# YoungSeng/QPGesture

Measured on AMD Instinct MI355X. Metric: matched gesture frames/sec (GestureKNN), higher is better.
Workload: dtype split-f16 products / f64 block sums + f64 re-evaluation; 1 GPU; 1 x 24 s clip (M=6 windows, Q=48 steps, 1440 frames each) per job vs speaker-10-class DB N_db=2048 windows (53248 candidates), shipped mode wavlm_feat(f32-bounded/f64-exact)+text(f32)+phase; n_db=2048, windows_per_clip=6, clips=1, clips_per_gpu=1, feature_dtype=f32, audio_precision=mixed, encode_batch=0, clips_in_flight=1, parallelism=single GPU, unsharded DB

## Files before the change

include/qpg.h:

```cpp
#ifndef QPG_H
#define QPG_H

#include <stddef.h>
#include <stdint.h>

#ifdef __cplusplus
extern "C" {
#endif

#define QPG_OK 0
#define QPG_EINVAL (-1)
#define QPG_EHIP (-2)
#define QPG_EUNSUP (-3)

typedef struct qpg_ctx qpg_ctx;

int qpg_version(void);
const char* qpg_build_id(void);
int qpg_ctx_create(int device, qpg_ctx** out);
int qpg_dev_kernarg(void);
int qpg_ctx_destroy(qpg_ctx* ctx);
#define QPG_OPT_GATE_DEDUP_FROM_CHAINS 0
#define QPG_OPT_TAKES_STAGES 1
#define QPG_OPT_COUNT 4
int qpg_ctx_set_option(qpg_ctx* ctx, int option, int value);
int qpg_ctx_get_option(qpg_ctx* ctx, int option, int* value);
int qpg_last_error(char* buf, size_t n);
int qpg_signal_i32(qpg_ctx*, void* stream, int32_t* dst, int32_t value);
int qpg_doorbell_wait(qpg_ctx*, void* stream, int32_t* counter, const int32_t* go, int32_t timeout_ms);


int qpg_wavlm_resample_f32(qpg_ctx*, void* stream, const float* x, int64_t N, int Tin, int F, int Tout, float* out);

int qpg_frame_norm2_f64(qpg_ctx*, void* stream, const float* x, int64_t rows, int F, double* out);

int qpg_audio_cand_norm2(qpg_ctx*, void* stream, const double* fn2, int N, int T, const int32_t* cand_t,
                         int G, int n_taps, int tap_stride, double* cn2);

int qpg_l2_normalize_rows_f32(qpg_ctx*, void* stream, const float* x, int64_t rows, int D, float* out);
int qpg_text_pack_queries_f32(qpg_ctx*, void* stream, const float* x, int M, int R, int D, const int32_t* q_win,
                              const int32_t* q_row, int Q, float* out);


int qpg_audio_pack_queries(qpg_ctx*, void* stream, const float* qbase, int M, int T, int F,
                           const int32_t* q_win, const int32_t* q_t, int Q, int n_taps, int tap_stride,
                           float* q32, double* qn2);

int qpg_audio_cosine_f64(qpg_ctx*, void* stream, const float* base, int N, int T, int F,
                         const int32_t* cand_t, int G, int n_taps, int tap_stride, const double* cn2,
                         const float* q32, const double* qn2, int Q, double* D, int64_t ldD);
int qpg_audio_cosine_f64_h(qpg_ctx*, void* stream, const void* base_f16, int N, int T, int F,
                           const int32_t* cand_t, int G, int n_taps, int tap_stride, const double* cn2,
                           const float* q32, const double* qn2, int Q, double* D, int64_t ldD);

#define QPG_AUDIO_MX_ERR 2.05e-6
int qpg_audio_cosine_mx(qpg_ctx*, void* stream, const float* base, int N, int T, int F, const int32_t* cand_t, int G,
                        int n_taps, int tap_stride, const double* cn2, const float* q32, const double* qn2, int Q,
                        void* D, int d_is_f32, int64_t ldD, int32_t* stats);

int qpg_audio_cosine_mx_h(qpg_ctx*, void* stream, const void* base_f16, int N, int T, int F, const int32_t* cand_t, int G,
                          int n_taps, int tap_stride, const double* cn2, const float* q32, const double* qn2, int Q,
                          void* D, int d_is_f32, int64_t ldD, int32_t* stats);

#define QPG_AUDIO_HL_ERR 1.3e-6
int qpg_audio_hl_supported(int T, int F, int G, int n_taps, int tap_stride, int cand_step);
int qpg_audio_pack_queries_hl(qpg_ctx*, void* stream, const float* qbase, int M, int T, int F, const int32_t* q_win,
                              const int32_t* q_t, int Q, int n_taps, int tap_stride, float* q32, double* qn2, void* image,
                              int64_t image_bytes);
int64_t qpg_audio_hl_db_bytes(int N, int F);
int64_t qpg_audio_hl_query_bytes(int Q, int F);
int qpg_audio_hl_pack_db(qpg_ctx*, void* stream, const float* base, int N, int T, int F, int G, int n_taps, int tap_stride,
                         int cand_step, void* image, int64_t image_bytes);
int qpg_audio_hl_pack_queries(qpg_ctx*, void* stream, const float* q32, int Q, int F, void* image, int64_t image_bytes);
int qpg_clip_pack_hl(qpg_ctx*, void* stream, const float* qbase, int M, int T, int F, const int32_t* q_win,
                     const int32_t* q_t, int Q, int n_taps, int tap_stride, float* q32, double* qn2, void* image,
                     int64_t image_bytes, const float* text_ctx, int Mt, int R, int Dt, const int32_t* tq_win,
                     const int32_t* tq_row, int Qt, float* qn_out, void* cols_image, int64_t cols_bytes);
int qpg_audio_cosine_hl(qpg_ctx*, void* stream, const void* db_image, int N, int F, int G, const double* cn2,
                        const void* q_image, const double* qn2, int Q, void* D, int d_is_f32, int64_t ldD, int32_t* stats);
int qpg_audio_hl1_supported(int T, int F, int G, int n_taps, int tap_stride, int cand_step);
int64_t qpg_audio_hl1_db_bytes(int N, int F);
int qpg_audio_hl1_pack_db(qpg_ctx*, void* stream, const void* base_f16, int N, int T, int F, int G, int n_taps,
                          int tap_stride, int cand_step, void* image, int64_t image_bytes);
int qpg_audio_cosine_hl1(qpg_ctx*, void* stream, const void* db_image, int N, int F, int G, const double* cn2,
                         const void* q_image, const double* qn2, int Q, void* D, int d_is_f32, int64_t ldD, int32_t* stats);
int qpg_probe_mfma_f16_tile(qpg_ctx*, void* stream, const void* a, const void* b, const float* c, int tiles, float* out);

int qpg_text_pack_candidates_f32(qpg_ctx*, void* stream, const float* x, int N, int R, int Dm,
                                 const int32_t* cand_r, int G, float* xt);

int qpg_text_cosine_f32(qpg_ctx*, void* stream, const float* xt, int64_t C, int Dm, const float* qn, int Q,
                        float* D, int64_t ldD);

int64_t qpg_text_percode_ws_bytes(int64_t C, int Q, int K, int tiles_per_chunk);
int qpg_text_percode_f32(qpg_ctx*, void* stream, const float* xt, int64_t C, int Dm, const int16_t* cand_code, int K,
                         const float* qn, int Q, int tiles_per_chunk, int32_t idx_base, float absent, void* ws,
                         int64_t ws_bytes, float* out_dist, int32_t* out_idx, int16_t* out_rank, int32_t* out_nn);
int qpg_text_pack_candidates_f16(qpg_ctx*, void* stream, const float* x, int N, int R, int Dm, const int32_t* cand_r,
                                 int G, void* xh, float* nrm);
int qpg_text_percode_f16(qpg_ctx*, void* stream, const void* xh, const float* nrm, int64_t C, int Dm,
                         const int16_t* cand_code, int K, const float* qn, int Q, int32_t idx_base, float absent,
                         void* ws, int64_t ws_bytes, float* out_dist, int32_t* out_idx, int16_t* out_rank,
                         int32_t* out_nn);

int64_t qpg_hl_rows_bytes(int64_t R, int D);
int64_t qpg_hl_cols_bytes(int Q, int D);
int qpg_hl_pack_rows(qpg_ctx*, void* stream, const float* xs, int64_t R, int D, void* image, int64_t image_bytes);
int qpg_hl_pack_cols(qpg_ctx*, void* stream, const float* qn, int Q, int D, void* image, int64_t image_bytes);
int qpg_hl_prepare_queries(qpg_ctx*, void* stream, const float* q, int Q, int D, float* qn_out, void* cols_image,
                           int64_t image_bytes, float* qperm_out);
int qpg_hl_gemm_distance(qpg_ctx*, void* stream, const void* rows_image, int64_t R, int D, const void* cols_image, int Q,
                         float* Dm, int64_t ldD, float* tile_min, int64_t ldT);
int qpg_hl_gemm_tilemin(qpg_ctx*, void* stream, const void* rows_image, int64_t R, int D, const void* cols_image, int Q,
                        float band, float* tile_min, uint16_t* tile_mask, int64_t ldT);
int qpg_hl_gemm_tilemin_h(qpg_ctx*, void* stream, const void* rows_image, int64_t R, int D, const void* cols_image, int Q,
                          float band, float* tile_min_t, uint16_t* tile_mask_t, int64_t ldQ);
int qpg_perm32_rows_f32(qpg_ctx*, void* stream, const float* x, int64_t R, int D, float* y);
int qpg_percode_select_bycode_f32(qpg_ctx*, void* stream, const float* tile_min_t, const uint16_t* tile_mask_t, int64_t ldQ,
                                  int Q, int64_t R, const int16_t* row_code, const int32_t* row_index,
                                  const int32_t* zero_row, const int32_t* code_tile, int K, float band,
                                  const float* qn_perm, const float* xs_perm, int D, float absent, float* out_dist,
                                  int32_t* out_idx, int16_t* out_rank, int32_t* out_nn, int32_t* stats, int32_t idx_base);
int qpg_percode_select_sorted_f32(qpg_ctx*, void* stream, const float* Dm, int64_t ldD, const float* tile_min,
                                  const uint16_t* tile_mask , int64_t ldT,
                                  int Q, int64_t R, const int16_t* row_code, const int32_t* row_index,
                                  const int32_t* zero_row, const int32_t* code_tile, int K, float band, const float* qn,
                                  const float* xs, int D, float absent, float* out_dist, int32_t* out_idx,
                                  int16_t* out_rank, int32_t* out_nn, int32_t* stats, int32_t idx_base, int q_block,
                                  int64_t block_stride);

int qpg_wavvq_lev_f32(qpg_ctx*, void* stream, const int32_t* sym_db, int N, int T, const int32_t* cand_t, int G,
                      const int32_t* tap_off, int n_taps, const int32_t* sym_q, int Mq, int Tq,
                      const int32_t* q_win, const int32_t* q_t, int Q, float* D, int64_t ldD);

int qpg_percode_select_f64(qpg_ctx*, void* stream, const double* D, int64_t ldD, int Q, const int16_t* cand_code,
                           int64_t C, int K, double absent, int32_t idx_base, double* out_dist, int32_t* out_idx,
                           int16_t* out_rank, int q_block, int64_t block_stride);
int qpg_percode_select_f32(qpg_ctx*, void* stream, const float* D, int64_t ldD, int Q, const int16_t* cand_code,
                           int64_t C, int K, float absent, int32_t idx_base, float* out_dist, int32_t* out_idx,
                           int16_t* out_rank, int q_block, int64_t block_stride);

int qpg_percode_select_guarded_f64(qpg_ctx*, void* stream, const double* D, int64_t ldD, int Q, const int16_t* cand_code,
                                   int64_t C, int K, double absent, int32_t idx_base, double* out_dist, int32_t* out_idx,
                                   int16_t* out_rank, int q_block, int64_t block_stride, const float* base, int T, int F,
                                   const int32_t* cand_t, int G, int n_taps, int tap_stride, const float* q32, double eps,
                                   int32_t* stats, int base_is_f16);

int64_t qpg_percode_select_exact_ws_bytes(int Q, int64_t C, int K);
int qpg_percode_select_exact_f64(qpg_ctx*, void* stream, const double* D, int64_t ldD, int Q, const int16_t* cand_code,
                                 int64_t C, int K, double absent, int32_t idx_base, double* out_dist, int32_t* out_idx,
                                 int16_t* out_rank, int q_block, int64_t block_stride, const float* base, int T, int F,
                                 const int32_t* cand_t, int G, int n_taps, int tap_stride, const float* q32, double eps,
                                 int32_t* stats, int base_is_f16, void* ws, int64_t ws_bytes);

int qpg_percode_select_mixed_f64(qpg_ctx*, void* stream, const void* D, int d_is_f32, int64_t ldD, int Q, const int16_t* cand_code,
                                 int64_t C, int K, double absent, int32_t idx_base, double* out_dist, int32_t* out_idx,
                                 int16_t* out_rank, int q_block, int64_t block_stride, const float* base, int T, int F,
                                 const int32_t* cand_t, int G, int n_taps, int tap_stride, const float* q32,
                                 const double* qn2, const double* cn2, double eps1, double eps2, int32_t* stats,
                                 void* ws, int64_t ws_bytes, int base_is_f16);
int64_t qpg_percode_select_mixed_ws_bytes(int Q, int K);
int64_t qpg_percode_select_mixed_ws_stride(int K);
int qpg_percode_select_mixed_f64_cut(qpg_ctx*, void* stream, const void* D, int d_is_f32, int64_t ldD, int Q,
                                     const int16_t* cand_code, int64_t C, int K, double absent, int32_t idx_base,
                                     double* out_dist, int32_t* out_idx, int16_t* out_rank, int q_block, int64_t block_stride,
                                     const float* base, int T, int F, const int32_t* cand_t, int G, int n_taps,
                                     int tap_stride, const float* q32, const double* qn2, const double* cn2, double eps1,
                                     double eps2, int32_t* stats, void* ws, int64_t ws_bytes, int base_is_f16,
                                     const int16_t* pos_rank_t, const int16_t* freq_rank, int top_n, int probe);

int64_t qpg_merge_mixed_ws_bytes(int Q, int K, int fl_cap);
int qpg_merge_mixed_phase1_f64(qpg_ctx*, void* stream, const void* recv, int W, int64_t src_stride, int64_t dist_off,
                               int64_t idx_off, int Q, int K, double absent, double eps1, int R, void* req,
                               int64_t req_stride, void* ws, int64_t ws_bytes, int32_t* stats, int fl_cap,
                               int64_t flag_off);
int qpg_shard_refine_f64(qpg_ctx*, void* stream, const void* req_recv, int W, int64_t req_stride, int R, int q_stride,
                         int64_t cand_base, const float* base, int base_is_f16, int T, int F, const int32_t* cand_t, int G,
                         int n_taps, int tap_stride, const float* q32, const double* qn2, const double* cn2, void* resp,
                         int64_t resp_stride, int reference_arithmetic, int32_t* stats, int Rq);
int qpg_flags_stamp(qpg_ctx*, void* stream, void* buf, int nblk, int64_t stride, int64_t off, const int32_t* stats);
int qpg_flags_gather(qpg_ctx*, void* stream, const void* buf, int nblk, int64_t stride, int64_t off, int32_t* stats);
int qpg_merge_mixed_phase2_f64(qpg_ctx*, void* stream, const void* recv, int W, int64_t src_stride, int64_t idx_off, int Q,
                               int K, double absent, const void* ws, int64_t ws_bytes, const void* resp_recv,
                               int64_t resp_stride, double* out_dist, int32_t* out_idx, int16_t* out_rank, int32_t* stats,
                               int fl_cap, double eps2);

int qpg_merge_select_f64(qpg_ctx*, void* stream, const void* recv, int W, int64_t src_stride, int64_t dist_off,
                         int64_t idx_off, int Q, int K, double absent, double* out_dist, int32_t* out_idx,
                         int16_t* out_rank, double eps2, int32_t* stats);
int qpg_merge_select_f32(qpg_ctx*, void* stream, const void* recv, int W, int64_t src_stride, int64_t dist_off,
                         int64_t idx_off, int Q, int K, float absent, float* out_dist, int32_t* out_idx,
                         int16_t* out_rank);

int qpg_rank_rows_f64(qpg_ctx*, void* stream, const double* d, int Q, int K, int16_t* out);
int qpg_rank_rows_f32(qpg_ctx*, void* stream, const float* d, int Q, int K, int16_t* out);


int qpg_l2_table_f32(qpg_ctx*, void* stream, const float* sig, int K, int Dm, float* out);

#define QPG_MODE_AUD_TXT 0
#define QPG_MODE_AUD 1
#define QPG_MODE_TXT 2
#define QPG_MODE_SERIAL_WALK 0x100
#define QPG_MODE_PREFUSED 0x200

int qpg_match_steps(qpg_ctx*, void* stream, const int16_t* aud_rank, const int32_t* aud_idx,
                    const int16_t* txt_rank, const int32_t* txt_idx, const int16_t* pos_rank,
                    const int16_t* freq_rank, const int32_t* code, int code_ld, const int32_t* aud_cidx,
                    const int32_t* aud_pslot, int Ga, const int32_t* txt_cidx, const int32_t* txt_pslot, int Gt,
                    const float* phase, int Tp, int mode, int M, int steps, int K, int seed_code,
                    const float* seed_phase, int32_t* gate_tables, int32_t* out_codes, float* out_phase,
                    int32_t* out_vote, int32_t* out_status, const int32_t* guard_flags);
int qpg_match_steps_batch(qpg_ctx*, void* stream, const int16_t* aud_rank, const int32_t* aud_idx, const int16_t* txt_rank,
                          const int32_t* txt_idx, const int16_t* pos_rank, const int16_t* freq_rank, const int32_t* code,
                          int code_ld, const int32_t* aud_cidx, const int32_t* aud_pslot, int Ga, const int32_t* txt_cidx,
                          const int32_t* txt_pslot, int Gt, const float* phase, int Tp, int mode, int M, int steps, int K,
                          int n_chains, const int32_t* seed_codes, const float* seed_phase, int32_t* gate_tables,
                          int32_t* out_codes, float* out_phase, int32_t* out_vote, int32_t* out_status,
                          int64_t status_stride, const int32_t* guard_flags);
#define QPG_TAKES_MAX 65536
size_t qpg_match_steps_takes_ws_bytes(int n_takes, int M, int steps);
int qpg_match_steps_takes(qpg_ctx*, void* stream, const int16_t* aud_rank, const int32_t* aud_idx, const int16_t* txt_rank,
                          const int32_t* txt_idx, const int16_t* pos_rank, const int16_t* freq_rank, const int32_t* code,
                          int code_ld, const int32_t* aud_cidx, const int32_t* aud_pslot, int Ga, const int32_t* txt_cidx,
                          const int32_t* txt_pslot, int Gt, const float* phase, int Tp, int mode, int M, int steps, int K,
                          int n_takes, const int32_t* seed_codes, const float* seed_phase, int32_t* gate_tables,
                          int32_t* out_codes, float* out_phase, int32_t* out_vote, int32_t* out_status,
                          int64_t status_stride, const int32_t* guard_flags, void* workspace, size_t workspace_bytes);
int qpg_fuse_best_ranked(qpg_ctx*, void* stream, const int16_t* rank, const int32_t* idx, const int16_t* pos_rank,
                         const int16_t* freq_rank, int Q, int K, int32_t* T);

typedef struct qpg_comm qpg_comm;
int qpg_comm_unique_id(void* id, int64_t id_bytes);
int qpg_comm_create(qpg_ctx*, const void* id, int64_t id_bytes, int rank, int world, qpg_comm** out);
int qpg_comm_destroy(qpg_comm*);
int qpg_comm_allgather(qpg_ctx*, void* stream, qpg_comm*, const void* send, void* recv, int64_t bytes);
int qpg_comm_alltoall(qpg_ctx*, void* stream, qpg_comm*, const void* send, void* recv, int64_t bytes);
int qpg_comm_allreduce_max_i32(qpg_ctx*, void* stream, qpg_comm*, int32_t* buf, int64_t count);
int qpg_allreduce_min_u64(qpg_ctx*, void* stream, qpg_comm*, uint64_t* buf, int64_t count);
int qpg_pack_min_u64(qpg_ctx*, void* stream, const float* dist, const int32_t* idx, int64_t n, uint64_t* packed);
int qpg_unpack_min_u64(qpg_ctx*, void* stream, const uint64_t* packed, int64_t n, float absent, float* dist, int32_t* idx);


int qpg_conv1d_f32(qpg_ctx*, void* stream, const float* x, int B, int T_in, int Cin, const float* w,
                   const float* bias, int taps, int Cin_pad, int Cout, int Cout_pad, int in_stride, int in_offset,
                   int dil, int T_out, int out_stride, int out_offset, int T_y, const float* residual, int relu_in,
                   int relu_out, float* y, float* ws, int64_t ws_floats);

int qpg_convt_f32(qpg_ctx*, void* stream, const float* x, int B, int T_in, int Cx, const float* wt, const float* bias,
                  int taps, int Cin_pad, int Cout, int Cout_pad, int in_stride, int in_offset, int dil, int T_out,
                  int out_stride, int out_offset, int T_y, const float* residual, int relu_in, int relu_out, float* y);
int qpg_convt_pair_f32(qpg_ctx*, void* stream, const float* x, int B, int T_in, int Cx, const float* wt0,
                       const float* bias0, int in_offset0, int out_offset0, const float* wt1, const float* bias1,
                       int in_offset1, int out_offset1, int taps, int Cin_pad, int Cout, int Cout_pad, int in_stride,
                       int dil, int T_out, int out_stride, int T_y, float* y);
int qpg_tpack_f32(qpg_ctx*, void* stream, const float* w, int taps, int Cin_pad, int Cout_pad, int nb, float* out);
int qpg_pad_channels_f32(qpg_ctx*, void* stream, const float* x, int64_t R, int C, int Cp, float* y);
int qpg_resblock_f32(qpg_ctx*, void* stream, const float* x, int B, int T, int dil, const float* wpack,
                     const float* b1, const float* b2, float* y, float* hidden);

int qpg_vq_argmin_f32(qpg_ctx*, void* stream, const float* z, const float* dot, const float* kk, int64_t R, int E,
                      int K, int64_t* ids, float* dmin, float* dsecond);

int qpg_vq_gather_f32(qpg_ctx*, void* stream, const float* k, const int64_t* ids, int64_t R, int E, int K, float* out,
                      int32_t* status);

#define QPG_CONV16_WEXP_FROM_IMAGE 0x7fff
int64_t qpg_conv16_image_bytes(int taps, int Cin, int Cout);
int qpg_conv16_pack_weights(qpg_ctx*, void* stream, const float* w, int taps, int Cin, int Cin_pad_w, int Cout, int Cout_pad_w,
                            void* image, int64_t image_bytes);
int qpg_conv16_f32(qpg_ctx*, void* stream, const float* x, int B, int T_in, int Cx, int Cin, const void* image, int w_exp,
                   const float* bias, int taps, int Cout, int in_stride, int in_offset, int dil, int T_out, int out_stride,
                   int out_offset, int T_y, const float* residual, int relu_in, int relu_out, float* y, int32_t* status);

#define QPG_VQ_MAX_DOWN 4
#define QPG_VQ_MAX_DEPTH 4
typedef struct {
  const float* w;
  const float* b;
  int32_t taps, cin, cin_pad, cout, cout_pad;
  const float* wt;
} qpg_conv_desc;
typedef struct {
  int32_t in_dim, width, emb, bins, down_t, depth, growth, reverse_dec;
  qpg_conv_desc enc_down[QPG_VQ_MAX_DOWN];
  qpg_conv_desc enc_res[QPG_VQ_MAX_DOWN][QPG_VQ_MAX_DEPTH][2];
  qpg_conv_desc enc_out;
  qpg_conv_desc dec_in;
  qpg_conv_desc dec_res[QPG_VQ_MAX_DOWN][QPG_VQ_MAX_DEPTH][2];
  qpg_conv_desc dec_up_even[QPG_VQ_MAX_DOWN];
  qpg_conv_desc dec_up_odd[QPG_VQ_MAX_DOWN];
  qpg_conv_desc dec_out;
  qpg_conv_desc kT;
  const float* k;
  const float* kk;
  const float* enc_res_pack[QPG_VQ_MAX_DOWN][QPG_VQ_MAX_DEPTH];
  const float* dec_res_pack[QPG_VQ_MAX_DOWN][QPG_VQ_MAX_DEPTH];
} qpg_vq_model;

int64_t qpg_vq_workspace_floats(const qpg_vq_model* m, int B, int T);
int qpg_vq_encode_f32(qpg_ctx*, void* stream, const qpg_vq_model* m, const float* x, int B, int T, float* ws,
                      int64_t ws_floats, int64_t* ids, float* latent, float* margin);
int qpg_vq_decode_f32(qpg_ctx*, void* stream, const qpg_vq_model* m, const int64_t* ids, int B, int L, float* ws,
                      int64_t ws_floats, float* out, int32_t* status);

int qpg_pose_to_euler_f64(qpg_ctx*, void* stream, const float* poses, int64_t T, int J, const double* mean,
                          const double* stdc, const double* sg_mid, const double* sg_head, const double* sg_tail, int W,
                          double* euler, int32_t* status);

#define QPG_PAE_CHANNELS 135
#define QPG_PAE_MID 15
#define QPG_PAE_EMBED 8
#define QPG_PAE_TIME 240
#define QPG_PAE_HALO 120
#define QPG_PAE_WS_STRIDE 136
#define QPG_PAE_MAX_CHUNK (1 << 22)
#define QPG_PAE_OFF_W1 0
#define QPG_PAE_OFF_BN1 522240
#define QPG_PAE_OFF_W2 522288
#define QPG_PAE_OFF_BN2 583728
#define QPG_PAE_OFF_FC 583776
#define QPG_PAE_OFF_FCBN 587616
#define QPG_PAE_OFF_FREQ 587664
#define QPG_PAE_OFF_TPI 587784
#define QPG_PAE_PARAM_FLOATS 587792
int qpg_pae_phase_f32(qpg_ctx*, void* stream, const float* params, const double* pose, const double* mean,
                      const double* stdc, const int64_t* clip_off, int n_clips, int64_t n_total, int64_t frame0,
                      int64_t n_frames, float* ws, int64_t ws_floats, float* out, float* v_out, float* latent_out);

#define QPG_PAET_OFF_TPI 0
#define QPG_PAET_OFF_ARGS 1
#define QPG_PAET_OFF_FREQS 241
#define QPG_PAET_TRAINABLE 361
#define QPG_PAET_OFF_CONV1_W 361
#define QPG_PAET_OFF_CONV1_B 486361
#define QPG_PAET_OFF_BN1 486376
#define QPG_PAET_OFF_CONV2_W 486406
#define QPG_PAET_OFF_CONV2_B 515206
#define QPG_PAET_OFF_BN2 515214
#define QPG_PAET_OFF_FC 515230
#define QPG_PAET_OFF_FCBN 519086
#define QPG_PAET_OFF_DECONV1_W 519118
#define QPG_PAET_OFF_DECONV1_B 547918
#define QPG_PAET_OFF_BN3 547933
#define QPG_PAET_OFF_DECONV2_W 547963
#define QPG_PAET_OFF_DECONV2_B 1033963
#define QPG_PAET_PARAM_FLOATS 1034098
#define QPG_PAET_ST_BN1 0
#define QPG_PAET_ST_BN2 30
#define QPG_PAET_ST_FCBN 46
#define QPG_PAET_ST_BN3 78
#define QPG_PAET_STATS_FLOATS 108
#define QPG_PAET_MAX_BATCH 65536
#define QPG_PAET_SLABS 16
int qpg_pae_train_ws_floats(qpg_ctx*, void* stream, int batch, int64_t* floats);
int qpg_pae_train_forward_f32(qpg_ctx*, void* stream, const float* params, float* stats, const float* poses,
                              int64_t n_frames, const int64_t* starts, int batch, int train, float* ws,
                              int64_t ws_floats, double* loss);
int qpg_pae_train_backward_f32(qpg_ctx*, void* stream, const float* params, int batch, float* ws, int64_t ws_floats,
                               float* grads);
int qpg_pae_adamw_f32(qpg_ctx*, void* stream, float* p, const float* g, float* m, float* v, int64_t n, double lr,
                      double weight_decay, double beta1, double beta2, double eps, int64_t step);

int64_t qpg_vq_reduce_ws_bytes(void);

int qpg_vq_loss_f32(qpg_ctx*, void* stream, const float* x_out, const float* x_target, int B, int T, int C,
                    const float* commit_loss, float w_commit, float w_reg, float w_vel, float w_acc, void* ws,
                    int64_t ws_bytes, float* out6);
int qpg_vq_loss_grad_f32(qpg_ctx*, void* stream, const float* x_out, const float* x_target, int B, int T, int C,
                         float w_reg, float w_vel, float w_acc, float upstream, float* d_x_out);

int qpg_vq_latent_stats_f32(qpg_ctx*, void* stream, const float* z, const float* zq, const float* dmin, int64_t R,
                            int E, void* ws, int64_t ws_bytes, float* out3);
int qpg_vq_commit_grad_f32(qpg_ctx*, void* stream, const float* z, const float* zq, int64_t R, int E, float scale,
                           const float* d_zq, float* d_z);

int64_t qpg_vq_code_sums_ws_bytes(int64_t R, int E, int K);
int qpg_vq_code_sums_f32(qpg_ctx*, void* stream, const float* z, const int64_t* ids, int64_t R, int E, int K,
                         float* batch_sum, float* batch_elem, void* ws, int64_t ws_bytes);
int qpg_vq_ema_update_f32(qpg_ctx*, void* stream, float* k, float* k_sum, float* k_elem, const float* batch_sum,
                          const float* batch_elem, const float* k_rand, float mu, float threshold, int K, int E,
                          float* kT, int ldkT, float* kk, void* ws, int64_t ws_bytes, float* out4);
int qpg_vq_code_norms_f32(qpg_ctx*, void* stream, const float* k, int K, int E, float* kk);

int qpg_adam_step_f32(qpg_ctx*, void* stream, float* param, const float* grad, float* exp_avg, float* exp_avg_sq,
                      int64_t n, float lr, float beta1, float beta2, float eps, int64_t step);

int qpg_conv1d_bwd_data_f32(qpg_ctx*, void* stream, const float* dy, int B, int T_in, int C_dy, const float* w_fwd,
                            int taps, int fwd_Cin, int fwd_Cin_pad, int fwd_Cout_pad, int tap_base, int tap_step,
                            int in_stride, int in_offset, int dil, int T_out, int out_stride, int out_offset, int T_y,
                            const float* gate, const float* residual, float* dx, float* ws, int64_t ws_floats);
int64_t qpg_conv1d_wgrad_ws_floats(int taps, int Cin_pad, int Cout_pad, int splits);
int qpg_conv1d_bwd_weight_f32(qpg_ctx*, void* stream, const float* x, int B, int T_in, int Cin, const float* dy,
                              int taps, int Cin_pad, int Cout, int Cout_pad, int in_stride, int in_offset, int dil,
                              int T_out, int out_stride, int out_offset, int T_y, int relu_in, float* dw, float* db,
                              int accumulate_bias, float* ws, int64_t ws_floats);

#ifdef QPG_DEBUG_HOOKS
int qpg_debug_gemm64_waves(int nw);
int qpg_debug_convt_shape(int nq, int pd);
int qpg_debug_convt_opts(int deep_ring, int xcd_map);
#endif

#ifdef __cplusplus
}
#endif
#endif
```

qpgesture_amd/csrc/qpg_common.h:

```cpp
#pragma once
#include <hip/hip_runtime.h>
#include <stdint.h>
#include <stdio.h>
#include <string.h>

#include "../../include/qpg.h"

struct qpg_ctx {
  int device;
  int n_cu;
  float* zeros;
  bool select_lds_raised;
  int opt[QPG_OPT_COUNT];
};

#ifdef QPG_DEBUG_HOOKS
#define QPG_HOOK_VAR(type, name, value) static type name = value
#else
#define QPG_HOOK_VAR(type, name, value) static constexpr type name = value
#endif

void qpg_set_error(const char* fmt, ...);

#define QPG_REQUIRE(cond, ...)      \
  do {                              \
    if (!(cond)) {                  \
      qpg_set_error(__VA_ARGS__);   \
      return QPG_EINVAL;            \
    }                               \
  } while (0)

#define QPG_LAUNCH_CHECK(name)                                                \
  do {                                                                        \
    hipError_t e_ = hipGetLastError();                                        \
    if (e_ != hipSuccess) {                                                   \
      qpg_set_error("%s: launch failed: %s", name, hipGetErrorString(e_));    \
      return QPG_EHIP;                                                        \
    }                                                                         \
  } while (0)

static inline hipStream_t qpg_stream(void* s) { return reinterpret_cast<hipStream_t>(s); }

typedef double f64x4 __attribute__((ext_vector_type(4)));
typedef float f32x4 __attribute__((ext_vector_type(4)));
typedef float f32x16 __attribute__((ext_vector_type(16)));

#pragma clang fp contract(off)
__device__ __forceinline__ float f_mul(float a, float b) { return a * b; }
__device__ __forceinline__ float f_add(float a, float b) { return a + b; }
__device__ __forceinline__ float f_sub(float a, float b) { return a - b; }
__device__ __forceinline__ float f_div(float a, float b) { return a / b; }
__device__ __forceinline__ float f_sqrt(float a) { return __builtin_sqrtf(a); }
__device__ __forceinline__ double f_mul(double a, double b) { return a * b; }
__device__ __forceinline__ double f_add(double a, double b) { return a + b; }
__device__ __forceinline__ double f_sub(double a, double b) { return a - b; }
__device__ __forceinline__ double f_div(double a, double b) { return a / b; }

__device__ __forceinline__ double cosine_from_dot(double dot, double qn2, double cn2) {
  const double tiny = 10.0 * 2.220446049250313e-16;
  double nq = sqrt(qn2), nc = sqrt(cn2);
  bool zq = nq < tiny, zc = nc < tiny;
  if (zq || zc) {
    double a = zq ? qn2 : 1.0, b = zc ? cn2 : 1.0;
    double cross = dot / ((zq ? 1.0 : nq) * (zc ? 1.0 : nc));
    return 0.5 * (a + b - 2.0 * cross);
  }
  return 1.0 - dot / (nq * nc);
}


__host__ __device__ __forceinline__ int rank_sort_pow2(int K) {
  int p = 2;
  while (p < K) p <<= 1;
  return p;
}
__device__ __forceinline__ unsigned long long rank_sort_key(double d) {
  const long long b = __double_as_longlong(d + 0.0);
  return b < 0 ? ~(unsigned long long)b : ((unsigned long long)b | 0x8000000000000000ull);
}
__device__ __forceinline__ unsigned long long rank_sort_key(float d) {
  const unsigned int b = __float_as_uint(d + 0.0f);
  return (unsigned long long)((b >> 31) ? ~b : (b | 0x80000000u));
}
template <int PJ>
__device__ __forceinline__ int lane_xor(int x) {
  if (PJ == 1) return __builtin_amdgcn_update_dpp(x, x, 0xB1, 0xf, 0xf, false);
  if (PJ == 2) return __builtin_amdgcn_update_dpp(x, x, 0x4E, 0xf, 0xf, false);
  if (PJ == 4) {
    const int t = __builtin_amdgcn_update_dpp(x, x, 0x104, 0xf, 0x5, false);
    return __builtin_amdgcn_update_dpp(t, x, 0x114, 0xf, 0xa, false);
  }
  if (PJ == 8) return __builtin_amdgcn_update_dpp(x, x, 0x128, 0xf, 0xf, false);
  if (PJ == 16) {
    const auto r = __builtin_amdgcn_permlane16_swap(x, x, false, false);
    return (threadIdx.x & 16) ? r[0] : r[1];
  }
  const auto r = __builtin_amdgcn_permlane32_swap(x, x, false, false);
  return (threadIdx.x & 32) ? r[0] : r[1];
}
template <int PJ>
__device__ __forceinline__ void lane_xor_pair(unsigned long long k0, unsigned long long k1, int c0, int c1,
                                              unsigned long long& p0, unsigned long long& p1, int& q0, int& q1) {
  const unsigned int a0 = (unsigned int)lane_xor<PJ>((int)(unsigned int)k0);
  const unsigned int a1 = (unsigned int)lane_xor<PJ>((int)(unsigned int)(k0 >> 32));
  const unsigned int a2 = (unsigned int)lane_xor<PJ>((int)(unsigned int)k1);
  const unsigned int a3 = (unsigned int)lane_xor<PJ>((int)(unsigned int)(k1 >> 32));
  q0 = lane_xor<PJ>(c0);
  q1 = lane_xor<PJ>(c1);
  p0 = ((unsigned long long)a1 << 32) | a0;
  p1 = ((unsigned long long)a3 << 32) | a2;
}

struct RankPair {
  unsigned long long k0, k1;
  int c0, c1;
};
__device__ __forceinline__ bool rank_gt(unsigned long long ka, int ca, unsigned long long kb, int cb) {
  return ka > kb || (ka == kb && ca > cb);
}
template <int J>
__device__ __forceinline__ void bitonic_chain(RankPair& e, int i0, int k, unsigned long long* skey, int* scode) {
  if constexpr (J == 0) {
    return;
  } else {
    if (J < k) {
      const bool up = (i0 & k) == 0;
      if constexpr (J == 1) {
        if (rank_gt(e.k0, e.c0, e.k1, e.c1) == up) {
          const unsigned long long tk = e.k0; e.k0 = e.k1; e.k1 = tk;
          const int tc = e.c0; e.c0 = e.c1; e.c1 = tc;
        }
      } else {
        unsigned long long p0, p1;
        int q0, q1;
        if constexpr (J / 2 < 64) {
          lane_xor_pair<J / 2>(e.k0, e.k1, e.c0, e.c1, p0, p1, q0, q1);
        } else {
          __syncthreads();
          skey[i0] = e.k0; skey[i0 + 1] = e.k1; scode[i0] = e.c0; scode[i0 + 1] = e.c1;
          __syncthreads();
          const int o0 = i0 ^ J;
          p0 = skey[o0]; p1 = skey[o0 + 1]; q0 = scode[o0]; q1 = scode[o0 + 1];
        }
        const bool keep_min = ((i0 & J) == 0) == up;
        if (rank_gt(e.k0, e.c0, p0, q0) == keep_min) { e.k0 = p0; e.c0 = q0; }
        if (rank_gt(e.k1, e.c1, p1, q1) == keep_min) { e.k1 = p1; e.c1 = q1; }
      }
    }
    bitonic_chain<J / 2>(e, i0, k, skey, scode);
  }
}
template <int KP, typename T, typename F>
__device__ __forceinline__ void block_sorted_ranks_unrolled(const T* v, int K, unsigned long long* skey, int* scode,
                                                            F&& emit) {
  const int tid = threadIdx.x;
  if ((tid & ~63) * 2 >= KP) {
    for (int k = 256; k <= KP; k <<= 1)
      for (int j = k >> 1; j >= 128; j >>= 1) {
        __syncthreads();
        __syncthreads();
      }
    return;
  }
  const int i0 = 2 * tid;
  RankPair e;
  e.k0 = i0 < K ? rank_sort_key(v[i0]) : ~0ull;
  e.k1 = i0 + 1 < K ? rank_sort_key(v[i0 + 1]) : ~0ull;
  e.c0 = i0;
  e.c1 = i0 + 1;
  for (int k = 2; k <= KP; k <<= 1) bitonic_chain<KP / 2>(e, i0, k, skey, scode);
  if (e.c0 < K) emit(e.c0, i0);
  if (e.c1 < K) emit(e.c1, i0 + 1);
}

template <typename T, typename F>
__device__ __forceinline__ void block_sorted_ranks(const T* v, int K, unsigned long long* skey, int* scode, F&& emit) {
  const int tid = threadIdx.x, nt = blockDim.x;
  const int Kp = rank_sort_pow2(K);
  if (Kp >= 128 && Kp <= 2 * nt && Kp <= 2048) {
    switch (Kp) {
      case 128: block_sorted_ranks_unrolled<128>(v, K, skey, scode, emit); break;
      case 256: block_sorted_ranks_unrolled<256>(v, K, skey, scode, emit); break;
      case 512: block_sorted_ranks_unrolled<512>(v, K, skey, scode, emit); break;
      case 1024: block_sorted_ranks_unrolled<1024>(v, K, skey, scode, emit); break;
      default: block_sorted_ranks_unrolled<2048>(v, K, skey, scode, emit); break;
    }
    return;
  }
  for (int i = tid; i < Kp; i += nt) {
    skey[i] = i < K ? rank_sort_key(v[i]) : ~0ull;
    scode[i] = i;
  }
  __syncthreads();
  for (int k = 2; k <= Kp; k <<= 1)
    for (int j = k >> 1; j > 0; j >>= 1) {
      for (int i = tid; i < (Kp >> 1); i += nt) {
        const int lo = ((i & ~(j - 1)) << 1) | (i & (j - 1));
        const int hi = lo + j;
        const unsigned long long ka = skey[lo], kb = skey[hi];
        const int ca = scode[lo], cb = scode[hi];
        const bool gt = ka > kb || (ka == kb && ca > cb);
        if (gt == ((lo & k) == 0)) {
          skey[lo] = kb; skey[hi] = ka;
          scode[lo] = cb; scode[hi] = ca;
        }
      }
      __syncthreads();
    }
  for (int r = tid; r < K; r += nt) emit(scode[r], r);
}
```

qpgesture_amd/csrc/qpg_core.hip:

```cpp
#include <stdarg.h>

#include "qpg_common.h"
#include <stdlib.h>

static thread_local char g_err[512] = "";

void qpg_set_error(const char* fmt, ...) {
  va_list ap;
  va_start(ap, fmt);
  vsnprintf(g_err, sizeof(g_err), fmt, ap);
  va_end(ap);
}

extern "C" int qpg_version(void) { return 109; }

#ifndef QPG_BUILD_ID
#define QPG_BUILD_ID "unstamped"
#endif
static const char g_build_id[] = "QPG_BUILD_ID=" QPG_BUILD_ID;
extern "C" const char* qpg_build_id(void) { return g_build_id + 13; }

extern "C" int qpg_dev_kernarg(void) {
  const char* e = getenv("HIP_FORCE_DEV_KERNARG");
  return (e && e[0] == '1') ? 1 : 0;
}

extern "C" int qpg_last_error(char* buf, size_t n) {
  if (!buf || n == 0) return QPG_EINVAL;
  strncpy(buf, g_err, n - 1);
  buf[n - 1] = 0;
  return QPG_OK;
}

extern "C" int qpg_ctx_create(int device, qpg_ctx** out) {
  QPG_REQUIRE(out != nullptr, "qpg_ctx_create: out is null");
  int n = 0;
  if (hipGetDeviceCount(&n) != hipSuccess || device < 0 || device >= n) {
    qpg_set_error("qpg_ctx_create: no HIP device %d (count %d)", device, n);
    return QPG_EHIP;
  }
  hipDeviceProp_t p;
  if (hipGetDeviceProperties(&p, device) != hipSuccess) {
    qpg_set_error("qpg_ctx_create: hipGetDeviceProperties failed");
    return QPG_EHIP;
  }
  qpg_ctx* c = new qpg_ctx;
  c->device = device;
  c->n_cu = p.multiProcessorCount;
  c->zeros = nullptr;
  c->select_lds_raised = false;
  for (int i = 0; i < QPG_OPT_COUNT; ++i) c->opt[i] = 0;
  c->opt[QPG_OPT_GATE_DEDUP_FROM_CHAINS] = 1;
  c->opt[QPG_OPT_TAKES_STAGES] = 7;
  int prev = 0;
  (void)hipGetDevice(&prev);
  const bool ok = hipSetDevice(device) == hipSuccess && hipMalloc(reinterpret_cast<void**>(&c->zeros), 4096) == hipSuccess &&
                  hipMemset(c->zeros, 0, 4096) == hipSuccess;
  (void)hipSetDevice(prev);
  if (!ok) {
    qpg_set_error("qpg_ctx_create: could not allocate the context's zero page on device %d", device);
    delete c;
    return QPG_EHIP;
  }
  *out = c;
  return QPG_OK;
}

extern "C" int qpg_ctx_set_option(qpg_ctx* ctx, int option, int value) {
  QPG_REQUIRE(ctx != nullptr, "qpg_ctx_set_option: null context");
  QPG_REQUIRE(option >= 0 && option < QPG_OPT_COUNT, "qpg_ctx_set_option: unknown option %d", option);
  if (option == QPG_OPT_GATE_DEDUP_FROM_CHAINS) QPG_REQUIRE(value >= 0, "qpg_ctx_set_option: gate_dedup_from_chains >= 0");
  ctx->opt[option] = value;
  return QPG_OK;
}

extern "C" int qpg_ctx_get_option(qpg_ctx* ctx, int option, int* value) {
  QPG_REQUIRE(ctx != nullptr && value != nullptr, "qpg_ctx_get_option: null pointer");
  QPG_REQUIRE(option >= 0 && option < QPG_OPT_COUNT, "qpg_ctx_get_option: unknown option %d", option);
  *value = ctx->opt[option];
  return QPG_OK;
}

extern "C" int qpg_ctx_destroy(qpg_ctx* ctx) {
  if (ctx && ctx->zeros) (void)hipFree(ctx->zeros);
  delete ctx;
  return QPG_OK;
}

__global__ void signal_i32_kernel(int32_t* dst, int32_t value) {
  __hip_atomic_store(dst, value, __ATOMIC_RELEASE, __HIP_MEMORY_SCOPE_SYSTEM);
}

extern "C" int qpg_signal_i32(qpg_ctx* ctx, void* stream, int32_t* dst, int32_t value) {
  QPG_REQUIRE(ctx && dst && (reinterpret_cast<uintptr_t>(dst) % 4) == 0, "qpg_signal_i32: null or misaligned destination");
  hipLaunchKernelGGL(signal_i32_kernel, dim3(1), dim3(1), 0, qpg_stream(stream), dst, value);
  QPG_LAUNCH_CHECK("signal_i32_kernel");
  return QPG_OK;
}

__global__ void doorbell_wait_kernel(int32_t* __restrict__ counter, const int32_t* __restrict__ go, int32_t timeout_ms) {
  const int32_t seq = atomicAdd(counter, 1) + 1;
  const long long t0 = wall_clock64();
  const long long limit = (long long)timeout_ms * 100000ll;
  while (__hip_atomic_load(go, __ATOMIC_RELAXED, __HIP_MEMORY_SCOPE_SYSTEM) - seq < 0) {
    if (wall_clock64() - t0 > limit) break;
    __builtin_amdgcn_s_sleep(16);
  }
  __atomic_thread_fence(__ATOMIC_ACQUIRE);
}

extern "C" int qpg_doorbell_wait(qpg_ctx* ctx, void* stream, int32_t* counter, const int32_t* go, int32_t timeout_ms) {
  QPG_REQUIRE(ctx && counter && go && timeout_ms > 0 && timeout_ms <= 60000, "qpg_doorbell_wait: bad argument (timeout 1..60000 ms)");
  hipLaunchKernelGGL(doorbell_wait_kernel, dim3(1), dim3(1), 0, qpg_stream(stream), counter, go, timeout_ms);
  QPG_LAUNCH_CHECK("doorbell_wait_kernel");
  return QPG_OK;
}

__global__ __launch_bounds__(256) void frame_norm2_kernel(const float* __restrict__ x, int64_t rows, int F,
                                                          double* __restrict__ out) {
  const int lane = threadIdx.x & 63;
  const int64_t row = (int64_t)blockIdx.x * 4 + (threadIdx.x >> 6);
  if (row >= rows) return;
  const float* p = x + row * F;
  double s = 0.0;
  if ((F & 3) == 0) {
    for (int e = lane * 4; e < F; e += 256) {
      f32x4 v = *reinterpret_cast<const f32x4*>(p + e);
      s += (double)v.x * v.x + (double)v.y * v.y + (double)v.z * v.z + (double)v.w * v.w;
    }
  } else {
    for (int e = lane; e < F; e += 64) s += (double)p[e] * p[e];
  }
  for (int o = 32; o > 0; o >>= 1) s += __shfl_down(s, o, 64);
  if (lane == 0) out[row] = s;
}

extern "C" int qpg_frame_norm2_f64(qpg_ctx* ctx, void* stream, const float* x, int64_t rows, int F, double* out) {
  QPG_REQUIRE(ctx && x && out && rows >= 0 && F > 0, "qpg_frame_norm2_f64: bad argument");
  if (rows == 0) return QPG_OK;
  hipLaunchKernelGGL(frame_norm2_kernel, dim3((unsigned)((rows + 3) / 4)), dim3(256), 0, qpg_stream(stream), x, rows,
                     F, out);
  QPG_LAUNCH_CHECK("frame_norm2_kernel");
  return QPG_OK;
}

__global__ void audio_cand_norm2_kernel(const double* __restrict__ fn2, int N, int T, const int32_t* __restrict__ cand_t,
                                        int G, int n_taps, int tap_stride, double* __restrict__ cn2) {
  int64_t i = (int64_t)blockIdx.x * blockDim.x + threadIdx.x;
  if (i >= (int64_t)N * G) return;
  int j = (int)(i / G), g = (int)(i % G);
  int t0 = cand_t[g];
  double s = 0.0;
  for (int k = 0; k < n_taps; ++k) {
    int t = t0 + k * tap_stride;
    if (t < T) s += fn2[(int64_t)j * T + t];
  }
  cn2[i] = s;
}

extern "C" int qpg_audio_cand_norm2(qpg_ctx* ctx, void* stream, const double* fn2, int N, int T,
                                    const int32_t* cand_t, int G, int n_taps, int tap_stride, double* cn2) {
  QPG_REQUIRE(ctx && fn2 && cand_t && cn2 && N >= 0 && T > 0 && G > 0 && n_taps > 0 && tap_stride > 0,
              "qpg_audio_cand_norm2: bad argument");
  int64_t n = (int64_t)N * G;
  if (n == 0) return QPG_OK;
  hipLaunchKernelGGL(audio_cand_norm2_kernel, dim3((unsigned)((n + 255) / 256)), dim3(256), 0, qpg_stream(stream),
                     fn2, N, T, cand_t, G, n_taps, tap_stride, cn2);
  QPG_LAUNCH_CHECK("audio_cand_norm2_kernel");
  return QPG_OK;
}

template <bool GATHER>
__global__ __launch_bounds__(256) void l2_normalize_rows_kernel(const float* __restrict__ x, int64_t rows, int D,
                                                                float* __restrict__ out,
                                                                const int32_t* __restrict__ win,
                                                                const int32_t* __restrict__ row, int R) {
  const int64_t t = (int64_t)blockIdx.x * blockDim.x + threadIdx.x;
  int64_t r = t >> 2;
  const int l = (int)(t & 3);
  const bool live = r < rows;
  if (!live) r = rows - 1;
  const float* p = GATHER ? x + ((int64_t)win[r] * R + row[r]) * D : x + r * D;
  float a = 0.f;
  const int nfull = D >> 4;
  int g = 0;
  for (; g + 8 <= nfull; g += 8) {
    float v[32];
#pragma unroll
    for (int j = 0; j < 32; ++j) v[j] = p[(g + (j >> 2)) * 16 + (j & 3) * 4 + l];
#pragma unroll
    for (int j = 0; j < 8; ++j) {
#pragma unroll
      for (int u = 3; u >= 0; --u) a = f_add(f_mul(v[j * 4 + u], v[j * 4 + u]), a);
    }
  }
  for (; g < nfull; ++g) {
#pragma unroll
    for (int u = 3; u >= 0; --u) {
      const float v = p[g * 16 + u * 4 + l];
      a = f_add(f_mul(v, v), a);
    }
  }
  for (int i = nfull * 16; i < D; i += 4) {
    const float v = (i + l < D) ? p[i + l] : 0.f;
    a = f_add(f_mul(v, v), a);
  }
  const float o1 = __shfl_xor(a, 1, 64);
  const float pair = f_add(a, o1);
  const float o2 = __shfl_xor(pair, 2, 64);
  float n = f_sqrt(f_add(pair, o2));
  if (n < 10.f * 1.1920928955078125e-07f) n = 1.f;
  if (live) {
    float* o = out + r * D;
    int e = l;
    for (; e + 28 < D; e += 32) {
      float v[8];
#pragma unroll
      for (int j = 0; j < 8; ++j) v[j] = p[e + 4 * j];
#pragma unroll
      for (int j = 0; j < 8; ++j) o[e + 4 * j] = f_div(v[j], n);
    }
    for (; e < D; e += 4) o[e] = f_div(p[e], n);
  }
}

extern "C" int qpg_l2_normalize_rows_f32(qpg_ctx* ctx, void* stream, const float* x, int64_t rows, int D, float* out) {
  QPG_REQUIRE(ctx && x && out && rows >= 0 && D > 0, "qpg_l2_normalize_rows_f32: bad argument");
  if (rows == 0) return QPG_OK;
  hipLaunchKernelGGL(l2_normalize_rows_kernel<false>, dim3((unsigned)((rows * 4 + 255) / 256)), dim3(256), 0,
                     qpg_stream(stream), x, rows, D, out, (const int32_t*)nullptr, (const int32_t*)nullptr, 0);
  QPG_LAUNCH_CHECK("l2_normalize_rows_kernel");
  return QPG_OK;
}

extern "C" int qpg_text_pack_queries_f32(qpg_ctx* ctx, void* stream, const float* x, int M, int R, int D,
                                         const int32_t* q_win, const int32_t* q_row, int Q, float* out) {
  QPG_REQUIRE(ctx && x && q_win && q_row && out && M > 0 && R > 0 && D > 0 && Q >= 0,
              "qpg_text_pack_queries_f32: bad argument");
  if (Q == 0) return QPG_OK;
  hipLaunchKernelGGL(l2_normalize_rows_kernel<true>, dim3((unsigned)(((int64_t)Q * 4 + 255) / 256)), dim3(256), 0,
                     qpg_stream(stream), x, (int64_t)Q, D, out, q_win, q_row, R);
  QPG_LAUNCH_CHECK("l2_normalize_rows_kernel<gather>");
  return QPG_OK;
}

__global__ __launch_bounds__(256) void wavlm_resample_kernel(const float* __restrict__ x, int64_t N, int Tin, int F,
                                                             int Tout, float scale, float* __restrict__ out) {
  const int64_t row = blockIdx.x;
  const int64_t n = row / Tout;
  const int t = (int)(row - n * Tout);
  const float src = f_mul(scale, (float)t);
  int i0 = (int)src;
  if (i0 > Tin - 1) i0 = Tin - 1;
  const int i1 = i0 + 1 < Tin ? i0 + 1 : Tin - 1;
  const float l1 = f_sub(src, (float)i0), l0 = f_sub(1.f, l1);
  const float* p0 = x + (n * Tin + i0) * F;
  const float* p1 = x + (n * Tin + i1) * F;
  float* o = out + row * F;
  for (int e = threadIdx.x; e < F; e += blockDim.x) o[e] = fmaf(l0, p0[e], f_mul(l1, p1[e]));
}

extern "C" int qpg_wavlm_resample_f32(qpg_ctx* ctx, void* stream, const float* x, int64_t N, int Tin, int F, int Tout,
                                      float* out) {
  QPG_REQUIRE(ctx && x && out && N >= 0 && Tin > 0 && F > 0 && Tout > 0, "qpg_wavlm_resample_f32: bad argument");
  QPG_REQUIRE(N * Tout < 0x7fffffffll, "qpg_wavlm_resample_f32: too many rows for one launch");
  if (N == 0) return QPG_OK;
  const float scale = Tout > 1 ? (float)(Tin - 1) / (float)(Tout - 1) : 0.f;
  hipLaunchKernelGGL(wavlm_resample_kernel, dim3((unsigned)(N * Tout)), dim3(256), 0, qpg_stream(stream), x, N, Tin, F,
                     Tout, scale, out);
  QPG_LAUNCH_CHECK("wavlm_resample_kernel");
  return QPG_OK;
}
```

qpgesture_amd/csrc/qpg_tail.hip:

```cpp
#include "qpg_common.h"

__global__ __launch_bounds__(256) void l2_table_kernel(const float* __restrict__ sig, int K, int Dm,
                                                       float* __restrict__ out) {
  const int p = blockIdx.x;
  for (int c = threadIdx.x; c < K; c += blockDim.x) {
    double s = 0.0;
    for (int e = 0; e < Dm; ++e) {
      const float d = f_sub(sig[(int64_t)p * Dm + e], sig[(int64_t)c * Dm + e]);
      s += (double)d * (double)d;
    }
    out[(int64_t)p * K + c] = (c == p) ? __builtin_inff() : (float)sqrt(s);
  }
}

extern "C" int qpg_l2_table_f32(qpg_ctx* ctx, void* stream, const float* sig, int K, int Dm, float* out) {
  QPG_REQUIRE(ctx && sig && out && K > 0 && Dm > 0, "qpg_l2_table_f32: bad argument");
  hipLaunchKernelGGL(l2_table_kernel, dim3(K), dim3(256), 0, qpg_stream(stream), sig, K, Dm, out);
  QPG_LAUNCH_CHECK("l2_table_kernel");
  return QPG_OK;
}

__device__ __forceinline__ float lane4_sum(float v, int l) {
  const float o1 = __shfl_xor(v, 1, 64);
  const float pair = (l & 1) ? f_add(o1, v) : f_add(v, o1);
  const float o2 = __shfl_xor(pair, 2, 64);
  return (l & 2) ? f_add(o2, pair) : f_add(pair, o2);
}

struct ArgMin {
  double v;
  int i;
};
__device__ __forceinline__ ArgMin amin(ArgMin a, ArgMin b) {
  return (b.v < a.v || (b.v == a.v && b.i < a.i)) ? b : a;
}
__device__ __forceinline__ ArgMin wave_argmin(ArgMin m) {
#pragma unroll
  for (int o = 32; o > 0; o >>= 1) {
    ArgMin t{__shfl_xor(m.v, o, 64), __shfl_xor(m.i, o, 64)};
    m = amin(m, t);
  }
  return m;
}

#define QPG_KMAX_PER_LANE 16

__global__ __launch_bounds__(256) void fuse_best_kernel(const int16_t* __restrict__ rank0,
                                                        const int32_t* __restrict__ idx0,
                                                        const int16_t* __restrict__ rank1,
                                                        const int32_t* __restrict__ idx1,
                                                        const int16_t* __restrict__ pos_rank,
                                                        const int16_t* __restrict__ freq_rank, int Q, int K, int mode,
                                                        int32_t* __restrict__ T0, int32_t* __restrict__ T1) {
  const int lane = threadIdx.x & 63;
  const int64_t task = (int64_t)blockIdx.x * 4 + (threadIdx.x >> 6);
  if (task >= (int64_t)Q * K) return;
  const int q = (int)(task / K), p = (int)(task - (int64_t)q * K);
  if (mode == 0) {
    const int16_t* ra = rank0 + (int64_t)q * K;
    const int16_t* rt = rank1 + (int64_t)q * K;
    ArgMin ma{__builtin_inf(), 0x7fffffff}, mt{__builtin_inf(), 0x7fffffff};
#pragma unroll
    for (int i = 0; i < QPG_KMAX_PER_LANE; ++i) {
      const int c = lane + 64 * i;
      if (c < K) {
        const double pos_score = (double)pos_rank[(int64_t)p * K + c] + (double)freq_rank[c] * 0.05;
        ma = amin(ma, ArgMin{pos_score + (double)ra[c], c});
        mt = amin(mt, ArgMin{pos_score + (double)rt[c], c});
      }
    }
    ma = wave_argmin(ma);
    mt = wave_argmin(mt);
    if (lane == 0) {
      T0[task] = idx0[(int64_t)q * K + ma.i];
      T1[task] = idx1[(int64_t)q * K + mt.i];
    }
    return;
  }
  const int16_t* rk = (mode == 1 ? rank0 : rank1) + (int64_t)q * K;
  const int32_t* ix = (mode == 1 ? idx0 : idx1) + (int64_t)q * K;
  ArgMin m{__builtin_inf(), 0x7fffffff};
  double vals[QPG_KMAX_PER_LANE];
#pragma unroll
  for (int i = 0; i < QPG_KMAX_PER_LANE; ++i) {
    const int c = lane + 64 * i;
    vals[i] = __builtin_inf();
    if (c < K) {
      const double pos_score = (double)pos_rank[(int64_t)p * K + c] + (double)freq_rank[c] * 0.05;
      vals[i] = pos_score + (double)rk[c];
      m = amin(m, ArgMin{vals[i], c});
    }
  }
  m = wave_argmin(m);
  ArgMin m2{__builtin_inf(), 0x7fffffff};
#pragma unroll
  for (int i = 0; i < QPG_KMAX_PER_LANE; ++i) {
    const int c = lane + 64 * i;
    if (c < K && c != m.i) m2 = amin(m2, ArgMin{vals[i], c});
  }
  m2 = wave_argmin(m2);
  if (lane == 0) {
    T0[task] = ix[m.i];
    T1[task] = ix[m2.i];
  }
}


template <int PJ>
__device__ __forceinline__ ArgMin argmin_xchg(ArgMin m) {
  const unsigned long long b = (unsigned long long)__double_as_longlong(m.v);
  const unsigned int lo = (unsigned int)lane_xor<PJ>((int)(unsigned int)b);
  const unsigned int hi = (unsigned int)lane_xor<PJ>((int)(unsigned int)(b >> 32));
  return ArgMin{__longlong_as_double((long long)(((unsigned long long)hi << 32) | lo)), lane_xor<PJ>(m.i)};
}

template <int NR>
__device__ __forceinline__ bool inverse_ranks(const int16_t* rk0, const int16_t* rk1, int K, int16_t* inv, int* bad) {
  const int tid = threadIdx.x;
  if (tid == 0) *bad = 0;
  for (int c = tid; c < NR * K; c += blockDim.x) inv[c] = -1;
  __syncthreads();
  for (int c = tid; c < K; c += blockDim.x) {
    const int r0 = rk0[c], r1 = NR == 2 ? rk1[c] : 0;
    if ((unsigned)r0 < (unsigned)K) inv[r0] = (int16_t)c; else *bad = 1;
    if (NR == 2) {
      if ((unsigned)r1 < (unsigned)K) inv[K + r1] = (int16_t)c; else *bad = 1;
    }
  }
  __syncthreads();
  for (int c = tid; c < NR * K; c += blockDim.x)
    if (inv[c] < 0) *bad = 1;
  __syncthreads();
  return *bad != 0;
}

__device__ __forceinline__ ArgMin ranked_scan(const int16_t* iv, const int16_t* rk, const int16_t* pr,
                                              const int16_t* freq_rank, int K, bool full, int l16) {
  ArgMin m{__builtin_inf(), 0x7fffffff};
  for (int base = 0; base < K; base += 64) {
    if (!full && (double)base > m.v) break;
    int c[4];
    double pv[4], fv[4], rr[4];
#pragma unroll
    for (int u = 0; u < 4; ++u) {
      const int r = base + 16 * u + l16;
      const bool ok = r < K;
      c[u] = ok ? (full ? r : (int)iv[r]) : -1;
      pv[u] = ok ? (double)pr[c[u]] : 0.0;
      fv[u] = ok ? (double)freq_rank[c[u]] : 0.0;
      rr[u] = ok ? (full ? (double)rk[c[u]] : (double)r) : 0.0;
    }
    ArgMin x{__builtin_inf(), 0x7fffffff};
#pragma unroll
    for (int u = 0; u < 4; ++u)
      if (c[u] >= 0) x = amin(x, ArgMin{(pv[u] + fv[u] * 0.05) + rr[u], c[u]});
    x = amin(x, argmin_xchg<8>(x));
    x = amin(x, argmin_xchg<4>(x));
    x = amin(x, argmin_xchg<2>(x));
    x = amin(x, argmin_xchg<1>(x));
    m = amin(m, x);
  }
  return m;
}

__global__ __launch_bounds__(256) void fuse_best_ranked_kernel(const int16_t* __restrict__ rank0,
                                                               const int32_t* __restrict__ idx0,
                                                               const int16_t* __restrict__ rank1,
                                                               const int32_t* __restrict__ idx1,
                                                               const int16_t* __restrict__ pos_rank,
                                                               const int16_t* __restrict__ freq_rank, int Q, int K,
                                                               int32_t* __restrict__ T0, int32_t* __restrict__ T1) {
  extern __shared__ __attribute__((aligned(16))) int16_t inv[];
  __shared__ int bad;
  const int tid = threadIdx.x, l16 = tid & 15;
  const int64_t task = (int64_t)blockIdx.x * 16 + (tid >> 4);
  const int q = (int)(((int64_t)blockIdx.x * 16) / K);
  const int p = (int)(task - (int64_t)q * K);
  const int16_t* ra = rank0 + (int64_t)q * K;
  const int16_t* rt = rank1 + (int64_t)q * K;
  const bool full = inverse_ranks<2>(ra, rt, K, inv, &bad);
  const int16_t* pr = pos_rank + (int64_t)p * K;
  const ArgMin ma = ranked_scan(inv, ra, pr, freq_rank, K, full, l16);
  const ArgMin mt = ranked_scan(inv + K, rt, pr, freq_rank, K, full, l16);
  if (l16 == 0) {
    T0[task] = idx0[(int64_t)q * K + ma.i];
    T1[task] = idx1[(int64_t)q * K + mt.i];
  }
}

__global__ __launch_bounds__(256) void fuse_best_ranked_one_kernel(const int16_t* __restrict__ rank,
                                                                   const int32_t* __restrict__ idx,
                                                                   const int16_t* __restrict__ pos_rank,
                                                                   const int16_t* __restrict__ freq_rank, int Q, int K,
                                                                   int32_t* __restrict__ T) {
  extern __shared__ __attribute__((aligned(16))) int16_t inv[];
  __shared__ int bad;
  const int tid = threadIdx.x, l16 = tid & 15;
  const int64_t task = (int64_t)blockIdx.x * 16 + (tid >> 4);
  const int q = (int)(((int64_t)blockIdx.x * 16) / K);
  const int p = (int)(task - (int64_t)q * K);
  const int16_t* rk = rank + (int64_t)q * K;
  const bool full = inverse_ranks<1>(rk, nullptr, K, inv, &bad);
  const ArgMin m = ranked_scan(inv, rk, pos_rank + (int64_t)p * K, freq_rank, K, full, l16);
  if (l16 == 0) T[task] = idx[(int64_t)q * K + m.i];
}

struct TailArgs {
  const int32_t* T0;
  const int32_t* T1;
  const int32_t* code;
  int code_ld;
  const int32_t* cidx0;
  const int32_t* pslot0;
  int G0;
  const int32_t* cidx1;
  const int32_t* pslot1;
  int G1;
  const float* phase;
  int Tp;
  int M, steps, step_codes, codes_per_window;
  int K;
  int seed_code;
  const float* seed_phase;
  const int32_t* seed_codes;
  int n_chains;
  int64_t status_stride;
  int32_t* out_codes;
  float* out_phase;
  int32_t* out_vote;
  int32_t* out_status;
  const int32_t* guard_flags;
};

__device__ __forceinline__ void write_status_pair(const TailArgs& A, const int& bad) {
  __threadfence_system();
  __syncthreads();
  if (threadIdx.x == 0) {
    A.out_status[0] = bad;
    __threadfence_system();
    A.out_status[1] = A.guard_flags ? A.guard_flags[0] : 0;
  }
}

__device__ __forceinline__ const float* chain_seed(const TailArgs& A, int chain, int* p) {
  *p = A.seed_codes ? A.seed_codes[chain] : A.seed_code;
  return A.seed_phase + (int64_t)chain * 128;
}

struct CandRegs {
  float2 head, tail;
  int pay;
  int absent;
};

__device__ __forceinline__ CandRegs load_cand(const TailArgs& A, int which, int ci, const int* s_cidx,
                                              const int* s_pslot, int lane) {
  const int G = which ? A.G1 : A.G0;
  const int cc = ci < 0 ? 0 : ci;
  const int j = cc / G, g = cc - j * G;
  const int ps = s_pslot[which * 64 + g];
  const float* b = A.phase + ((int64_t)j * A.Tp + ps) * 16;
  CandRegs r;
  r.absent = ci < 0;
  r.head = reinterpret_cast<const float2*>(b)[lane];
  r.tail = reinterpret_cast<const float2*>(b + 384)[lane];
  r.pay = A.code[(int64_t)j * A.code_ld + s_cidx[which * 64 + g] + (lane & 3)];
  return r;
}

__device__ __forceinline__ float einsum_sq_128_t(const float* vt, int l) {
  const f32x4* p = reinterpret_cast<const f32x4*>(vt + l * 32);
  float a = 0.f;
#pragma unroll
  for (int g = 0; g < 8; ++g) {
    const f32x4 x = p[g];
    a = f_add(f_mul(x.w, x.w), a);
    a = f_add(f_mul(x.z, x.z), a);
    a = f_add(f_mul(x.y, x.y), a);
    a = f_add(f_mul(x.x, x.x), a);
  }
  return lane4_sum(a, l);
}

__device__ __forceinline__ int tpos(int e) { return (e & 3) * 32 + (e >> 2); }

__global__ __launch_bounds__(64) void match_walk_kernel(TailArgs A) {
  extern __shared__ __attribute__((aligned(16))) int32_t tab[];
  __shared__ __attribute__((aligned(16))) float va[2][128], vb[2][128];
  __shared__ float nrm[4];
  __shared__ float score[2];
  __shared__ int wincodes[64];
  __shared__ int s_cidx[128], s_pslot[128];

  const int lane = threadIdx.x, K = A.K;
  int prev_code;
  float2 prev = reinterpret_cast<const float2*>(chain_seed(A, 0, &prev_code))[lane];
  if (lane < A.G0) {
    s_cidx[lane] = A.cidx0[lane];
    s_pslot[lane] = A.pslot0[lane];
  }
  if (lane < A.G1) {
    s_cidx[64 + lane] = A.cidx1[lane];
    s_pslot[64 + lane] = A.pslot1[lane];
  }
  int bad = 0;
  const float eps10 = 10.f * 1.1920928955078125e-07f;
  const int last_idx = A.codes_per_window - 1;
  const int e0 = 2 * lane;

  for (int w = 0; w < A.M; ++w) {
    const int n4 = A.steps * K / 4;
    __syncthreads();
    for (int t = 0; t < 2; ++t) {
      const int4* src = reinterpret_cast<const int4*>((t ? A.T1 : A.T0) + (int64_t)w * A.steps * K);
      int4* dst = reinterpret_cast<int4*>(tab + t * A.steps * K);
      for (int v = lane; v < n4; v += 64) dst[v] = src[v];
    }
    __syncthreads();
    CandRegs cur[2];
    cur[0] = load_cand(A, 0, tab[prev_code], s_cidx, s_pslot, lane);
    cur[1] = load_cand(A, 1, tab[A.steps * K + prev_code], s_cidx, s_pslot, lane);

    for (int s = 0; s < A.steps; ++s) {
      bad |= cur[0].absent | cur[1].absent;
#pragma unroll
      for (int k = 0; k < 2; ++k) {
        if (e0 >= 48) {
          va[k][tpos(e0 - 48)] = prev.x;
          va[k][tpos(e0 - 47)] = prev.y;
        }
        if (e0 >= 80) {
          vb[k][tpos(e0 - 80)] = prev.x;
          vb[k][tpos(e0 - 79)] = prev.y;
        }
        if (e0 < 48) {
          va[k][tpos(e0 + 80)] = cur[k].head.x;
          va[k][tpos(e0 + 81)] = cur[k].head.y;
        }
        if (e0 < 80) {
          vb[k][tpos(e0 + 48)] = cur[k].head.x;
          vb[k][tpos(e0 + 49)] = cur[k].head.y;
        }
      }
      CandRegs nxt[2][2];
      const bool spec = s + 1 < A.steps;
      if (spec) {
#pragma unroll
        for (int k = 0; k < 2; ++k) {
          const int pn = __shfl(cur[k].pay, 3, 64);
          nxt[k][0] = load_cand(A, 0, tab[(s + 1) * K + pn], s_cidx, s_pslot, lane);
          nxt[k][1] = load_cand(A, 1, tab[A.steps * K + (s + 1) * K + pn], s_cidx, s_pslot, lane);
        }
      }
      __syncthreads();
      if (lane < 16) {
        const int l = lane & 3, grp = lane >> 2;
        const float* v = (grp & 1) ? vb[grp >> 1] : va[grp >> 1];
        float n = f_sqrt(einsum_sq_128_t(v, l));
        if (n < eps10) n = 1.f;
        if (l == 0) nrm[grp] = n;
      }
      __syncthreads();
#pragma unroll
      for (int k = 0; k < 2; ++k) {
        const float na = nrm[2 * k], nb = nrm[2 * k + 1];
        const float2 xa = reinterpret_cast<const float2*>(va[k])[lane], xb = reinterpret_cast<const float2*>(vb[k])[lane];
        float2 d;
        d.x = f_sub(f_div(xa.x, na), f_div(xb.x, nb));
        d.y = f_sub(f_div(xa.y, na), f_div(xb.y, nb));
        reinterpret_cast<float2*>(va[k])[lane] = d;
      }
      __syncthreads();
      if (lane < 8) {
        const int l = lane & 3, k = lane >> 2;
        const float sc = f_mul(0.5f, einsum_sq_128_t(va[k], l));
        if (l == 0) score[k] = sc;
      }
      __syncthreads();
      const int fi = (score[1] < score[0]) ? 1 : 0;
      prev = fi ? cur[1].tail : cur[0].tail;
      reinterpret_cast<float2*>(A.out_phase + ((int64_t)w * A.steps + s) * 128)[lane] = prev;
      const int wpay = fi ? cur[1].pay : cur[0].pay;
      if (lane < A.step_codes) wincodes[s * A.step_codes + lane] = wpay;
      if (lane == 0) A.out_vote[w * A.steps + s] = fi;
      prev_code = __shfl(wpay, A.step_codes - 1, 64);
      if (spec) {
        cur[0] = fi ? nxt[1][0] : nxt[0][0];
        cur[1] = fi ? nxt[1][1] : nxt[0][1];
      }
    }
    __syncthreads();
    if (lane < A.codes_per_window) A.out_codes[(int64_t)w * A.codes_per_window + lane] = wincodes[lane];
    prev_code = wincodes[last_idx];
  }
  write_status_pair(A, bad);
}


struct GateGeom {
  int s_last, off_last;
};

__device__ __forceinline__ const float* cand_block(const TailArgs& A, int which, int ci, int* pay_base) {
  const int G = which ? A.G1 : A.G0;
  const int cc = ci < 0 ? 0 : ci;
  const int j = cc / G, g = cc - j * G;
  const int ps = (which ? A.pslot1 : A.pslot0)[g];
  *pay_base = j * A.code_ld + (which ? A.cidx1 : A.cidx0)[g];
  return A.phase + ((int64_t)j * A.Tp + ps) * 16;
}

__device__ __forceinline__ unsigned int gate_eval(const TailArgs& A, int q, int p, const float* prev, int lane) {
  const int K = A.K;
  const int k = (lane >> 2) & 1, l = lane & 3;
  const int ck = (k ? A.T1 : A.T0)[(int64_t)q * K + p];
  int pb_unused;
  const float* head = cand_block(A, k, ck, &pb_unused);
  float xa[32], xb[32];
  float sa = 0.f, sb = 0.f;
#pragma unroll
  for (int g = 0; g < 8; ++g) {
#pragma unroll
    for (int u = 3; u >= 0; --u) {
      const int e = g * 16 + u * 4 + l;
      const float va = e < 80 ? prev[48 + e] : head[e - 80];
      const float vb = e < 48 ? prev[80 + e] : head[e - 48];
      xa[g * 4 + u] = va;
      xb[g * 4 + u] = vb;
      sa = f_add(f_mul(va, va), sa);
      sb = f_add(f_mul(vb, vb), sb);
    }
  }
  const float eps10 = 10.f * 1.1920928955078125e-07f;
  float na = f_sqrt(lane4_sum(sa, l)), nb = f_sqrt(lane4_sum(sb, l));
  if (na < eps10) na = 1.f;
  if (nb < eps10) nb = 1.f;
  float sd = 0.f;
#pragma unroll
  for (int g = 0; g < 8; ++g) {
#pragma unroll
    for (int u = 3; u >= 0; --u) {
      const float d = f_sub(f_div(xa[g * 4 + u], na), f_div(xb[g * 4 + u], nb));
      sd = f_add(f_mul(d, d), sd);
    }
  }
  const float score = f_mul(0.5f, lane4_sum(sd, l));
  const float other = __shfl_xor(score, 4, 64);
  const float s0 = k ? other : score, s1 = k ? score : other;
  const int fi = (s1 < s0) ? 1 : 0;
  return (unsigned int)((p << 1) | fi);
}

__device__ __forceinline__ const float* gate_prev(const TailArgs& A, const GateGeom& geo, int s, int kp, int ci, int* p) {
  int pb;
  const float* prev = cand_block(A, kp, ci, &pb) + 384;
  *p = A.code[pb + (s == 0 ? geo.off_last : A.step_codes - 1)];
  return prev;
}

__global__ __launch_bounds__(256) void gate_table_kernel(TailArgs A, GateGeom geo, uint16_t* __restrict__ Gt) {
  const int K = A.K, Qc = A.M * A.steps, Q = Qc * A.n_chains;
  const int lane = threadIdx.x & 63;
  const int64_t task = ((int64_t)blockIdx.x * 256 + threadIdx.x) >> 3;
  const int64_t n_task = (int64_t)Q * 2 * K;
  const bool live = task < n_task;
  const int q = live ? (int)(task / (2 * K)) : 0;
  const int sigma = live ? (int)(task - (int64_t)q * 2 * K) : 0;
  const int chain = q / Qc;
  const bool first = q == chain * Qc;
  if (first && sigma != 0) return;
  const int s = q % A.steps;
  int p;
  const float* prev;
  if (first) {
    prev = chain_seed(A, chain, &p);
  } else {
    const int pp = sigma >> 1, kp = sigma & 1;
    const int ci = (kp ? A.T1 : A.T0)[(int64_t)(q - 1) * K + pp];
    prev = gate_prev(A, geo, s, kp, ci, &p);
  }
  const unsigned int g = gate_eval(A, q, p, prev, lane);
  if (live && (lane & 7) == 0) Gt[task] = (uint16_t)g;
}

#define GD_SLOTS 2048
#define GD_THREADS 1024
__global__ __launch_bounds__(GD_THREADS) void gate_table_dedup_kernel(TailArgs A, GateGeom geo, uint16_t* __restrict__ Gt) {
  __shared__ int key[GD_SLOTS];
  __shared__ unsigned short val[GD_SLOTS];
  __shared__ unsigned short ulist[GD_SLOTS];
  __shared__ int n_u;
  const int K = A.K, Qc = A.M * A.steps, tid = threadIdx.x, lane = tid & 63;
  const int q = blockIdx.x, chain = q / Qc, s = q % A.steps;
  uint16_t* out = Gt + (int64_t)q * 2 * K;
  if (q == chain * Qc) {
    if (tid < 8) {
      int p;
      const float* prev = chain_seed(A, chain, &p);
      const unsigned int g = gate_eval(A, q, p, prev, lane);
      if (tid == 0) out[0] = (uint16_t)g;
    }
    return;
  }
  for (int i = tid; i < GD_SLOTS; i += GD_THREADS) key[i] = 0;
  if (tid == 0) n_u = 0;
  __syncthreads();
  constexpr int PER = 2 * 512 / GD_THREADS;
  int slot[PER];
#pragma unroll
  for (int u = 0; u < PER; ++u) {
    const int sigma = u * GD_THREADS + tid;
    slot[u] = -1;
    if (sigma < 2 * K) {
      const int pp = sigma >> 1, kp = sigma & 1;
      const int ci = (kp ? A.T1 : A.T0)[(int64_t)(q - 1) * K + pp];
      const int kv = (((ci < 0 ? 0 : ci) << 1) | kp) + 1;
      unsigned int h = ((unsigned int)kv * 2654435761u) >> 21;
      for (;;) {
        const int old = atomicCAS(&key[h], 0, kv);
        if (old == 0) {
          ulist[atomicAdd(&n_u, 1)] = (unsigned short)h;
          break;
        }
        if (old == kv) break;
        h = (h + 1) & (GD_SLOTS - 1);
      }
      slot[u] = (int)h;
    }
  }
  __syncthreads();
  const int nu = n_u;
  for (int u = tid >> 3; u < nu; u += GD_THREADS >> 3) {
    const int h = ulist[u], kv = key[h] - 1;
    int p;
    const float* prev = gate_prev(A, geo, s, kv & 1, kv >> 1, &p);
    const unsigned int g = gate_eval(A, q, p, prev, lane);
    if ((lane & 7) == 0) val[h] = (unsigned short)g;
  }
  __syncthreads();
#pragma unroll
  for (int u = 0; u < PER; ++u)
    if (slot[u] >= 0) out[u * GD_THREADS + tid] = val[slot[u]];
}

#define QPG_CHASE_QMAX 2048

template <class Chase>
__device__ __forceinline__ void chase_windows(uint16_t* gl, const uint16_t* __restrict__ Gt, int M, int per_w, Chase chase) {
  const int tid = threadIdx.x, nt = blockDim.x;
  auto stage = [&](int w, int first, int step) {
    const int4* src = reinterpret_cast<const int4*>(Gt + (int64_t)w * per_w);
    int4* dst = reinterpret_cast<int4*>(gl + (size_t)(w & 1) * per_w);
    for (int v = first; v < per_w / 8; v += step) dst[v] = src[v];
  };
  stage(0, tid, nt);
  __syncthreads();
  for (int w = 0; w < M; ++w) {
    if (tid >= 64 && w + 1 < M) stage(w + 1, tid - 64, nt - 64);
    chase(w, gl + (size_t)(w & 1) * per_w);
    __syncthreads();
  }
}

__device__ __forceinline__ void walk_epilogue(const TailArgs& A, const uint16_t* sig, int* bad, int Q, int K) {
  const int tid = threadIdx.x, nt = blockDim.x;
  for (int i = tid; i < Q * 32; i += nt) {
    const int q = i >> 5, v = i & 31;
    const int sg = sig[q], p = sg >> 1, fi = sg & 1;
    const int ci = (fi ? A.T1 : A.T0)[(int64_t)q * K + p];
    int pb;
    const float* blk = cand_block(A, fi, ci, &pb) + 384;
    reinterpret_cast<f32x4*>(A.out_phase + (int64_t)q * 128)[v] = reinterpret_cast<const f32x4*>(blk)[v];
    if (v == 0) {
      A.out_vote[q] = fi;
      if (A.T0[(int64_t)q * K + p] < 0 || A.T1[(int64_t)q * K + p] < 0) *bad = 1;
    }
  }
  for (int i = tid; i < A.M * A.codes_per_window; i += nt) {
    const int w = i / A.codes_per_window, c = i - w * A.codes_per_window;
    const int q = w * A.steps + c / A.step_codes;
    const int sg = sig[q], p = sg >> 1, fi = sg & 1;
    const int ci = (fi ? A.T1 : A.T0)[(int64_t)q * K + p];
    int pb;
    cand_block(A, fi, ci, &pb);
    A.out_codes[i] = A.code[pb + c % A.step_codes];
  }
  write_status_pair(A, *bad);
}

__global__ __launch_bounds__(1024) void gate_chase_kernel(TailArgs A, const uint16_t* __restrict__ Gt) {
  extern __shared__ __attribute__((aligned(16))) uint16_t gl[];
  __shared__ uint16_t sig[QPG_CHASE_QMAX];
  __shared__ int bad_s;
  const int K = A.K, Q = A.M * A.steps, tid = threadIdx.x;
  const int per_w = A.steps * 2 * K;
  const int chain = blockIdx.x;
  const int64_t q0 = (int64_t)chain * Q;
  Gt += q0 * 2 * K;
  A.T0 += q0 * K;
  A.T1 += q0 * K;
  A.out_phase += q0 * 128;
  A.out_vote += q0;
  A.out_codes += (int64_t)chain * A.M * A.codes_per_window;
  A.out_status += (int64_t)chain * A.status_stride;
  if (tid == 0) bad_s = 0;
  int sigma = 0;
  chase_windows(gl, Gt, A.M, per_w, [&](int w, const uint16_t* g) {
    if (tid == 0) {
      for (int s = 0; s < A.steps; ++s) {
        sigma = (w == 0 && s == 0) ? g[0] : g[s * 2 * K + sigma];
        sig[w * A.steps + s] = (uint16_t)sigma;
      }
    }
  });
  walk_epilogue(A, sig, &bad_s, Q, K);
}

#define QPG_TAKES_PER_BLOCK 64
__host__ __device__ __forceinline__ int64_t takes_trail_off(int n_takes) { return ((int64_t)n_takes + 7) & ~(int64_t)7; }

__global__ __launch_bounds__(256) void takes_step0_kernel(TailArgs A, int n_takes, uint16_t* __restrict__ step0) {
  const int lane = threadIdx.x & 63;
  const int task = (int)(((int64_t)blockIdx.x * 256 + threadIdx.x) >> 3);
  const bool live = task < n_takes;
  const int take = live ? task : n_takes - 1;
  int p;
  const float* prev = chain_seed(A, take, &p);
  p = p < 0 ? 0 : (p >= A.K ? A.K - 1 : p);
  const unsigned int g = gate_eval(A, 0, p, prev, lane);
  if (live && (lane & 7) == 0) step0[take] = (uint16_t)g;
}

__global__ __launch_bounds__(1024) void gate_chase_takes_kernel(int M, int steps, int K, int n_takes,
                                                                const uint16_t* __restrict__ Gt,
                                                                const uint16_t* __restrict__ step0,
                                                                uint16_t* __restrict__ trail) {
  extern __shared__ __attribute__((aligned(16))) uint16_t gl[];
  const int tid = threadIdx.x;
  const int per_w = steps * 2 * K;
  const int take = blockIdx.x * QPG_TAKES_PER_BLOCK + tid;
  const bool chaser = tid < QPG_TAKES_PER_BLOCK && take < n_takes;
  int sigma = chaser ? step0[take] : 0;
  chase_windows(gl, Gt, M, per_w, [&](int w, const uint16_t* g) {
    if (chaser) {
      for (int s = 0; s < steps; ++s) {
        if (w | s) sigma = g[s * 2 * K + sigma];
        trail[(int64_t)(w * steps + s) * n_takes + take] = (uint16_t)sigma;
      }
    }
  });
}

__global__ __launch_bounds__(256) void takes_epilogue_kernel(TailArgs A, int n_takes, const uint16_t* __restrict__ trail) {
  __shared__ uint16_t sig[QPG_CHASE_QMAX];
  __shared__ int bad_s;
  const int K = A.K, Q = A.M * A.steps, tid = threadIdx.x, nt = blockDim.x;
  const int take = blockIdx.x;
  A.out_phase += (int64_t)take * Q * 128;
  A.out_vote += (int64_t)take * Q;
  A.out_codes += (int64_t)take * A.M * A.codes_per_window;
  A.out_status += (int64_t)take * A.status_stride;
  if (tid == 0) bad_s = 0;
  for (int q = tid; q < Q; q += nt) sig[q] = trail[(int64_t)q * n_takes + take];
  __syncthreads();
  walk_epilogue(A, sig, &bad_s, Q, K);
}

__global__ void status_only_kernel(int32_t* out_status, const int32_t* guard_flags) {
  out_status[0] = 0;
  out_status[1] = guard_flags ? guard_flags[0] : 0;
}

extern "C" int qpg_fuse_best_ranked(qpg_ctx* ctx, void* stream, const int16_t* rank, const int32_t* idx,
                                    const int16_t* pos_rank, const int16_t* freq_rank, int Q, int K, int32_t* T) {
  QPG_REQUIRE(ctx && rank && idx && pos_rank && freq_rank && T, "qpg_fuse_best_ranked: null pointer");
  QPG_REQUIRE(Q > 0 && K > 0 && (K % 16) == 0 && K <= 4096 && ((int64_t)Q * K) / 16 < 0x7fffffffll,
              "qpg_fuse_best_ranked: K %% 16 == 0, K <= 4096");
  hipLaunchKernelGGL(fuse_best_ranked_one_kernel, dim3((unsigned)(((int64_t)Q * K) / 16)), dim3(256), 2 * (size_t)K,
                     qpg_stream(stream), rank, idx, pos_rank, freq_rank, Q, K, T);
  QPG_LAUNCH_CHECK("fuse_best_ranked_one_kernel");
  return QPG_OK;
}

struct WalkGeom {
  int codes_per_window;
  GateGeom gate;
  size_t lds_cand;
  size_t lds_chase;
  bool tabulated;
};

static WalkGeom walk_geom(bool serial_walk, int steps, int K, int Qc) {
  WalkGeom g;
  g.codes_per_window = (steps * 4 < 30) ? steps * 4 : 30;
  const int last_idx = g.codes_per_window - 1;
  g.gate = GateGeom{last_idx / 4, last_idx % 4};
  g.lds_cand = (size_t)2 * steps * K * sizeof(int32_t);
  g.lds_chase = (size_t)2 * steps * 2 * K * sizeof(uint16_t);
  g.tabulated = !serial_walk && g.gate.s_last == steps - 1 && 2 * K <= 65536 && Qc <= QPG_CHASE_QMAX &&
                g.lds_chase <= 64 * 1024 && ((steps * 2 * K) % 8) == 0;
  return g;
}

static int walk_lds_ok(const char* name, const void* kernel, size_t dyn) {
  if (dyn <= 56 * 1024) return QPG_OK;
  hipFuncAttributes fa;
  if (hipFuncGetAttributes(&fa, kernel) != hipSuccess) {
    qpg_set_error("%s: cannot read the kernel's attributes", name);
    return QPG_EHIP;
  }
  if (fa.sharedSizeBytes + dyn > 64 * 1024 &&
      hipFuncSetAttribute(kernel, hipFuncAttributeMaxDynamicSharedMemorySize, (int)dyn) != hipSuccess) {
    qpg_set_error("%s: cannot raise the dynamic LDS limit to %zu bytes", name, dyn);
    return QPG_EHIP;
  }
  return QPG_OK;
}

struct WalkArgs {
  const int16_t* aud_rank; const int32_t* aud_idx; const int16_t* txt_rank; const int32_t* txt_idx;
  const int16_t* pos_rank; const int16_t* freq_rank; const int32_t* code; int code_ld;
  const int32_t* aud_cidx; const int32_t* aud_pslot; int Ga;
  const int32_t* txt_cidx; const int32_t* txt_pslot; int Gt;
  const float* phase; int Tp, mode, M, steps, K;
  const float* seed_phase; int32_t* gate_tables; int32_t* out_codes; float* out_phase; int32_t* out_vote;
  int32_t* out_status; const int32_t* guard_flags;
  int seed_code = 0;
  const int32_t* seed_codes = nullptr;
  int n_chains = 1;
  int64_t status_stride = 2;
  int n_takes = 0;
  void* takes_ws = nullptr;
  size_t takes_ws_bytes = 0;
};

static int match_steps_impl(qpg_ctx* ctx, void* stream, const WalkArgs& a) {
  const int M = a.M, steps = a.steps, K = a.K, n_chains = a.n_chains, n_takes = a.n_takes;
  QPG_REQUIRE(ctx && a.pos_rank && a.freq_rank && a.code && a.phase && a.seed_phase && a.gate_tables && a.out_codes &&
                  a.out_phase && a.out_vote && a.out_status,
              "qpg_match_steps: null pointer");
  QPG_REQUIRE(n_chains >= 1 && (n_chains == 1 || (a.seed_codes && a.status_stride >= 2)),
              "qpg_match_steps_batch: n_chains >= 1, device seed codes and a status stride >= 2");
  const bool serial_walk = (a.mode & QPG_MODE_SERIAL_WALK) != 0;
  const bool prefused = (a.mode & QPG_MODE_PREFUSED) != 0;
  const int mode = a.mode & ~(QPG_MODE_SERIAL_WALK | QPG_MODE_PREFUSED);
  QPG_REQUIRE(!prefused || mode == 0, "qpg_match_steps: QPG_MODE_PREFUSED goes with the two-modality mode");
  QPG_REQUIRE(mode >= 0 && mode <= 2, "qpg_match_steps: bad mode %d", mode);
  QPG_REQUIRE(mode == QPG_MODE_TXT || (a.aud_rank && a.aud_idx && a.aud_cidx && a.aud_pslot && a.Ga > 0),
              "qpg_match_steps: audio tables missing");
  QPG_REQUIRE(mode == QPG_MODE_AUD || (a.txt_rank && a.txt_idx && a.txt_cidx && a.txt_pslot && a.Gt > 0),
              "qpg_match_steps: text tables missing");
  QPG_REQUIRE(M >= 0 && steps > 0 && steps * 4 <= 64 && K > 0 && K <= 64 * QPG_KMAX_PER_LANE && (K % 4) == 0 &&
                  a.seed_code >= 0 && a.seed_code < K && a.Ga <= 64 && a.Gt <= 64,
              "qpg_match_steps: bad size");
  const int Qc = M * steps;
  const int Q = Qc * n_chains;
  const WalkGeom geo = walk_geom(serial_walk, steps, K, Qc);
  QPG_REQUIRE(geo.lds_cand <= 96 * 1024, "qpg_match_steps: steps*K too large for the LDS gate tables");
  if (M == 0) {
    hipLaunchKernelGGL(status_only_kernel, dim3(1), dim3(1), 0, qpg_stream(stream), a.out_status, a.guard_flags);
    QPG_LAUNCH_CHECK("status_only_kernel");
    return QPG_OK;
  }
  if (n_takes > 0 && !geo.tabulated) {
    qpg_set_error("qpg_match_steps_takes: the tabulated walk does not apply (serial walk asked for, or steps = %d / K = %d "
                  "/ %d steps per clip outside its geometry)", steps, K, Qc);
    return QPG_EUNSUP;
  }
  QPG_REQUIRE(n_takes <= 0 || (a.takes_ws && a.takes_ws_bytes >= qpg_match_steps_takes_ws_bytes(n_takes, M, steps)),
              "qpg_match_steps_takes: workspace too small (qpg_match_steps_takes_ws_bytes)");
  {
    int rc = QPG_OK;
    if (!geo.tabulated) rc = walk_lds_ok("match_walk_kernel", reinterpret_cast<const void*>(match_walk_kernel), geo.lds_cand);
    else if (n_takes > 0)
      rc = walk_lds_ok("gate_chase_takes_kernel", reinterpret_cast<const void*>(gate_chase_takes_kernel), geo.lds_chase);
    else rc = walk_lds_ok("gate_chase_kernel", reinterpret_cast<const void*>(gate_chase_kernel), geo.lds_chase);
    if (rc != QPG_OK) return rc;
  }
  int32_t* T0 = a.gate_tables;
  int32_t* T1 = a.gate_tables + (int64_t)Q * K;
  if (prefused) {
  } else if (mode == 0 && (K % 16) == 0 && K <= 4096) {
    hipLaunchKernelGGL(fuse_best_ranked_kernel, dim3((unsigned)(((int64_t)Q * K) / 16)), dim3(256), 4 * (size_t)K,
                       qpg_stream(stream), a.aud_rank, a.aud_idx, a.txt_rank, a.txt_idx, a.pos_rank, a.freq_rank, Q, K, T0,
                       T1);
    QPG_LAUNCH_CHECK("fuse_best_ranked_kernel");
  } else {
    dim3 grid((unsigned)(((int64_t)Q * K + 3) / 4), 1);
    hipLaunchKernelGGL(fuse_best_kernel, grid, dim3(256), 0, qpg_stream(stream), a.aud_rank, a.aud_idx, a.txt_rank,
                       a.txt_idx, a.pos_rank, a.freq_rank, Q, K, mode, T0, T1);
    QPG_LAUNCH_CHECK("fuse_best_kernel");
  }
  TailArgs A;
  A.T0 = T0; A.T1 = T1; A.code = a.code; A.code_ld = a.code_ld;
  const bool txt0 = (mode == QPG_MODE_TXT), txt1 = (mode != QPG_MODE_AUD);
  A.cidx0 = txt0 ? a.txt_cidx : a.aud_cidx; A.pslot0 = txt0 ? a.txt_pslot : a.aud_pslot; A.G0 = txt0 ? a.Gt : a.Ga;
  A.cidx1 = txt1 ? a.txt_cidx : a.aud_cidx; A.pslot1 = txt1 ? a.txt_pslot : a.aud_pslot; A.G1 = txt1 ? a.Gt : a.Ga;
  A.phase = a.phase; A.Tp = a.Tp; A.M = M; A.steps = steps; A.step_codes = 4;
  A.codes_per_window = geo.codes_per_window;
  A.K = K; A.seed_code = a.seed_code; A.seed_phase = a.seed_phase; A.seed_codes = a.seed_codes; A.n_chains = n_chains;
  A.status_stride = a.status_stride;
  A.out_codes = a.out_codes; A.out_phase = a.out_phase; A.out_vote = a.out_vote; A.out_status = a.out_status;
  A.guard_flags = a.guard_flags;
  if (!geo.tabulated) {
    QPG_REQUIRE(n_chains == 1, "qpg_match_steps_batch: the sequential walk takes one chain per call");
    hipLaunchKernelGGL(match_walk_kernel, dim3(1), dim3(64), geo.lds_cand, qpg_stream(stream), A);
    QPG_LAUNCH_CHECK("match_walk_kernel");
    return QPG_OK;
  }
  uint16_t* gtab = reinterpret_cast<uint16_t*>(a.gate_tables + (int64_t)2 * Q * K);
  const int64_t lanes = (int64_t)Q * 2 * K * 8;
  const int dedup_from = ctx->opt[QPG_OPT_GATE_DEDUP_FROM_CHAINS];
  if (dedup_from > 0 && n_chains >= dedup_from && K <= 512) {
    hipLaunchKernelGGL(gate_table_dedup_kernel, dim3((unsigned)Q), dim3(GD_THREADS), 0, qpg_stream(stream), A, geo.gate,
                       gtab);
    QPG_LAUNCH_CHECK("gate_table_dedup_kernel");
  } else {
    hipLaunchKernelGGL(gate_table_kernel, dim3((unsigned)((lanes + 255) / 256)), dim3(256), 0, qpg_stream(stream), A,
                       geo.gate, gtab);
    QPG_LAUNCH_CHECK("gate_table_kernel");
  }
  if (n_takes > 0) {
    uint16_t* step0 = reinterpret_cast<uint16_t*>(a.takes_ws);
    uint16_t* trail = step0 + takes_trail_off(n_takes);
    const int stages = ctx->opt[QPG_OPT_TAKES_STAGES];
    if (stages & 1) {
      hipLaunchKernelGGL(takes_step0_kernel, dim3((unsigned)(((int64_t)n_takes * 8 + 255) / 256)), dim3(256), 0,
                         qpg_stream(stream), A, n_takes, step0);
      QPG_LAUNCH_CHECK("takes_step0_kernel");
    }
    if (stages & 2) {
      hipLaunchKernelGGL(gate_chase_takes_kernel,
                         dim3((unsigned)((n_takes + QPG_TAKES_PER_BLOCK - 1) / QPG_TAKES_PER_BLOCK)), dim3(1024),
                         geo.lds_chase, qpg_stream(stream), M, steps, K, n_takes, (const uint16_t*)gtab,
                         (const uint16_t*)step0, trail);
      QPG_LAUNCH_CHECK("gate_chase_takes_kernel");
    }
    if (stages & 4) {
      hipLaunchKernelGGL(takes_epilogue_kernel, dim3((unsigned)n_takes), dim3(256), 0, qpg_stream(stream), A, n_takes,
                         (const uint16_t*)trail);
      QPG_LAUNCH_CHECK("takes_epilogue_kernel");
    }
    return QPG_OK;
  }
  hipLaunchKernelGGL(gate_chase_kernel, dim3(n_chains), dim3(1024), geo.lds_chase, qpg_stream(stream), A,
                     (const uint16_t*)gtab);
  QPG_LAUNCH_CHECK("gate_chase_kernel");
  return QPG_OK;
}

extern "C" int qpg_match_steps(qpg_ctx* ctx, void* stream, const int16_t* aud_rank, const int32_t* aud_idx,
                               const int16_t* txt_rank, const int32_t* txt_idx, const int16_t* pos_rank,
                               const int16_t* freq_rank, const int32_t* code, int code_ld, const int32_t* aud_cidx,
                               const int32_t* aud_pslot, int Ga, const int32_t* txt_cidx, const int32_t* txt_pslot,
                               int Gt, const float* phase, int Tp, int mode, int M, int steps, int K, int seed_code,
                               const float* seed_phase, int32_t* gate_tables, int32_t* out_codes, float* out_phase,
                               int32_t* out_vote, int32_t* out_status, const int32_t* guard_flags) {
  WalkArgs a{aud_rank, aud_idx, txt_rank, txt_idx, pos_rank, freq_rank, code, code_ld, aud_cidx, aud_pslot, Ga,
             txt_cidx, txt_pslot, Gt, phase, Tp, mode, M, steps, K, seed_phase, gate_tables, out_codes, out_phase,
             out_vote, out_status, guard_flags};
  a.seed_code = seed_code;
  return match_steps_impl(ctx, stream, a);
}

extern "C" int qpg_match_steps_batch(qpg_ctx* ctx, void* stream, const int16_t* aud_rank, const int32_t* aud_idx,
                                     const int16_t* txt_rank, const int32_t* txt_idx, const int16_t* pos_rank,
                                     const int16_t* freq_rank, const int32_t* code, int code_ld, const int32_t* aud_cidx,
                                     const int32_t* aud_pslot, int Ga, const int32_t* txt_cidx, const int32_t* txt_pslot,
                                     int Gt, const float* phase, int Tp, int mode, int M, int steps, int K,
                                     int n_chains, const int32_t* seed_codes, const float* seed_phase,
                                     int32_t* gate_tables, int32_t* out_codes, float* out_phase, int32_t* out_vote,
                                     int32_t* out_status, int64_t status_stride, const int32_t* guard_flags) {
  QPG_REQUIRE(M > 0 && seed_codes, "qpg_match_steps_batch: M > 0 and device seed codes");
  WalkArgs a{aud_rank, aud_idx, txt_rank, txt_idx, pos_rank, freq_rank, code, code_ld, aud_cidx, aud_pslot, Ga,
             txt_cidx, txt_pslot, Gt, phase, Tp, mode, M, steps, K, seed_phase, gate_tables, out_codes, out_phase,
             out_vote, out_status, guard_flags};
  a.seed_codes = seed_codes; a.n_chains = n_chains; a.status_stride = status_stride;
  return match_steps_impl(ctx, stream, a);
}

extern "C" size_t qpg_match_steps_takes_ws_bytes(int n_takes, int M, int steps) {
  if (n_takes < 1 || M < 1 || steps < 1) return 0;
  return sizeof(uint16_t) * (size_t)(takes_trail_off(n_takes) + (int64_t)M * steps * n_takes);
}

extern "C" int qpg_match_steps_takes(qpg_ctx* ctx, void* stream, const int16_t* aud_rank, const int32_t* aud_idx,
                                     const int16_t* txt_rank, const int32_t* txt_idx, const int16_t* pos_rank,
                                     const int16_t* freq_rank, const int32_t* code, int code_ld, const int32_t* aud_cidx,
                                     const int32_t* aud_pslot, int Ga, const int32_t* txt_cidx, const int32_t* txt_pslot,
                                     int Gt, const float* phase, int Tp, int mode, int M, int steps, int K,
                                     int n_takes, const int32_t* seed_codes, const float* seed_phase,
                                     int32_t* gate_tables, int32_t* out_codes, float* out_phase, int32_t* out_vote,
                                     int32_t* out_status, int64_t status_stride, const int32_t* guard_flags,
                                     void* workspace, size_t workspace_bytes) {
  QPG_REQUIRE(M > 0 && seed_codes && n_takes >= 1 && n_takes <= QPG_TAKES_MAX && status_stride >= 2,
              "qpg_match_steps_takes: M > 0, 1 <= n_takes <= %d, device seed codes and a status stride >= 2", QPG_TAKES_MAX);
  WalkArgs a{aud_rank, aud_idx, txt_rank, txt_idx, pos_rank, freq_rank, code, code_ld, aud_cidx, aud_pslot, Ga,
             txt_cidx, txt_pslot, Gt, phase, Tp, mode, M, steps, K, seed_phase, gate_tables, out_codes, out_phase,
             out_vote, out_status, guard_flags};
  a.seed_codes = seed_codes; a.status_stride = status_stride;
  a.n_takes = n_takes; a.takes_ws = workspace; a.takes_ws_bytes = workspace_bytes;
  return match_steps_impl(ctx, stream, a);
}
```

Before: 5.469 million frames/s.

## Stage gate tables in a multi-window LDS ring and stage fusion operands in LDS

```diff
diff --git a/include/qpg.h b/include/qpg.h
--- a/include/qpg.h
+++ b/include/qpg.h
@@ -22,6 +22,7 @@
 int qpg_ctx_destroy(qpg_ctx* ctx);
 #define QPG_OPT_GATE_DEDUP_FROM_CHAINS 0
 #define QPG_OPT_TAKES_STAGES 1
+#define QPG_OPT_CHASE_RING_WINDOWS 2
 #define QPG_OPT_COUNT 4
 int qpg_ctx_set_option(qpg_ctx* ctx, int option, int value);
 int qpg_ctx_get_option(qpg_ctx* ctx, int option, int* value);
@@ -220,6 +221,7 @@
                           int64_t status_stride, const int32_t* guard_flags);
 #define QPG_TAKES_MAX 65536
 size_t qpg_match_steps_takes_ws_bytes(int n_takes, int M, int steps);
+int qpg_match_steps_ring_windows(qpg_ctx*, int M, int steps, int K, int takes);
 int qpg_match_steps_takes(qpg_ctx*, void* stream, const int16_t* aud_rank, const int32_t* aud_idx, const int16_t* txt_rank,
                           const int32_t* txt_idx, const int16_t* pos_rank, const int16_t* freq_rank, const int32_t* code,
                           int code_ld, const int32_t* aud_cidx, const int32_t* aud_pslot, int Ga, const int32_t* txt_cidx,
diff --git a/qpgesture_amd/csrc/qpg_common.h b/qpgesture_amd/csrc/qpg_common.h
--- a/qpgesture_amd/csrc/qpg_common.h
+++ b/qpgesture_amd/csrc/qpg_common.h
@@ -11,6 +11,11 @@
   int n_cu;
   float* zeros;
   bool select_lds_raised;
+  int lds_per_block;
+  struct {
+    int static_bytes;
+    size_t granted;
+  } walk_lds[3];
   int opt[QPG_OPT_COUNT];
 };
 
diff --git a/qpgesture_amd/csrc/qpg_core.hip b/qpgesture_amd/csrc/qpg_core.hip
--- a/qpgesture_amd/csrc/qpg_core.hip
+++ b/qpgesture_amd/csrc/qpg_core.hip
@@ -49,6 +49,15 @@
   c->n_cu = p.multiProcessorCount;
   c->zeros = nullptr;
   c->select_lds_raised = false;
+  int lds = 0, lds_optin = 0;
+  if (hipDeviceGetAttribute(&lds, hipDeviceAttributeMaxSharedMemoryPerBlock, device) != hipSuccess) lds = 64 * 1024;
+  if (hipDeviceGetAttribute(&lds_optin, hipDeviceAttributeSharedMemPerBlockOptin, device) != hipSuccess) lds_optin = 0;
+  (void)hipGetLastError();
+  c->lds_per_block = lds_optin > lds ? lds_optin : lds;
+  for (auto& k : c->walk_lds) {
+    k.static_bytes = -1;
+    k.granted = 56 * 1024;
+  }
   for (int i = 0; i < QPG_OPT_COUNT; ++i) c->opt[i] = 0;
   c->opt[QPG_OPT_GATE_DEDUP_FROM_CHAINS] = 1;
   c->opt[QPG_OPT_TAKES_STAGES] = 7;
@@ -70,6 +79,8 @@
   QPG_REQUIRE(ctx != nullptr, "qpg_ctx_set_option: null context");
   QPG_REQUIRE(option >= 0 && option < QPG_OPT_COUNT, "qpg_ctx_set_option: unknown option %d", option);
   if (option == QPG_OPT_GATE_DEDUP_FROM_CHAINS) QPG_REQUIRE(value >= 0, "qpg_ctx_set_option: gate_dedup_from_chains >= 0");
+  if (option == QPG_OPT_CHASE_RING_WINDOWS)
+    QPG_REQUIRE(value == 0 || value >= 2, "qpg_ctx_set_option: chase_ring_windows is 0 (automatic) or >= 2");
   ctx->opt[option] = value;
   return QPG_OK;
 }
diff --git a/qpgesture_amd/csrc/qpg_tail.hip b/qpgesture_amd/csrc/qpg_tail.hip
--- a/qpgesture_amd/csrc/qpg_tail.hip
+++ b/qpgesture_amd/csrc/qpg_tail.hip
@@ -163,46 +163,99 @@
   return m;
 }
 
+typedef int i32x4 __attribute__((ext_vector_type(4)));
+struct FuseOps {
+  const int16_t *rk0, *rk1;
+  const int16_t* freq;
+  const int16_t* pos;
+  const int32_t *ix0, *ix1;
+};
+#define QPG_FUSE_STAGED_KMAX 1024
+
+template <int NR>
+__device__ __forceinline__ FuseOps stage_fusion(int16_t* st, const FuseOps& g, int K) {
+  const int n_r = K / 8, n_p = 2 * K, n_i = K / 4;
+  const int o_f = NR * n_r, o_p = o_f + n_r, o_i = o_p + n_p, n4 = o_i + NR * n_i;
+  const int nt = blockDim.x;
+  i32x4* dst = reinterpret_cast<i32x4*>(st);
+  constexpr int U = 6;
+  for (int base = threadIdx.x; base < n4; base += U * nt) {
+    i32x4 r[U];
+#pragma unroll
+    for (int u = 0; u < U; ++u) {
+      const int v = base + u * nt;
+      const void* src = g.rk0;
+      int o = 0;
+      if (v >= n4) {
+      } else if (v < o_f) {
+        const bool second = NR == 2 && v >= n_r;
+        src = second ? g.rk1 : g.rk0;
+        o = second ? v - n_r : v;
+      } else if (v < o_p) {
+        src = g.freq;
+        o = v - o_f;
+      } else if (v < o_i) {
+        src = g.pos;
+        o = v - o_p;
+      } else {
+        const bool second = NR == 2 && v >= o_i + n_i;
+        src = second ? g.ix1 : g.ix0;
+        o = v - o_i - (second ? n_i : 0);
+      }
+      r[u] = reinterpret_cast<const i32x4*>(src)[o];
+    }
+#pragma unroll
+    for (int u = 0; u < U; ++u)
+      if (base + u * nt < n4) dst[base + u * nt] = r[u];
+  }
+  const int32_t* ix = reinterpret_cast<const int32_t*>(st + (NR + 17) * K);
+  return FuseOps{st, st + K, st + NR * K, st + (NR + 1) * K, ix, ix + K};
+}
+
+template <int NR>
+__device__ __forceinline__ void fuse_tasks(const FuseOps& o, int K, int16_t* inv, int* bad, int32_t* T0, int32_t* T1) {
+  const int l16 = threadIdx.x & 15, grp = threadIdx.x >> 4;
+  const bool full = inverse_ranks<NR>(o.rk0, o.rk1, K, inv, bad);
+  const int16_t* pr = o.pos + grp * K;
+  const ArgMin ma = ranked_scan(inv, o.rk0, pr, o.freq, K, full, l16);
+  if (l16 == 0) T0[grp] = o.ix0[ma.i];
+  if (NR == 2) {
+    const ArgMin mt = ranked_scan(inv + K, o.rk1, pr, o.freq, K, full, l16);
+    if (l16 == 0) T1[grp] = o.ix1[mt.i];
+  }
+}
+
 __global__ __launch_bounds__(256) void fuse_best_ranked_kernel(const int16_t* __restrict__ rank0,
                                                                const int32_t* __restrict__ idx0,
                                                                const int16_t* __restrict__ rank1,
                                                                const int32_t* __restrict__ idx1,
                                                                const int16_t* __restrict__ pos_rank,
                                                                const int16_t* __restrict__ freq_rank, int Q, int K,
-                                                               int32_t* __restrict__ T0, int32_t* __restrict__ T1) {
+                                                               int staged, int32_t* __restrict__ T0,
+                                                               int32_t* __restrict__ T1) {
   extern __shared__ __attribute__((aligned(16))) int16_t inv[];
   __shared__ int bad;
-  const int tid = threadIdx.x, l16 = tid & 15;
-  const int64_t task = (int64_t)blockIdx.x * 16 + (tid >> 4);
-  const int q = (int)(((int64_t)blockIdx.x * 16) / K);
-  const int p = (int)(task - (int64_t)q * K);
-  const int16_t* ra = rank0 + (int64_t)q * K;
-  const int16_t* rt = rank1 + (int64_t)q * K;
-  const bool full = inverse_ranks<2>(ra, rt, K, inv, &bad);
-  const int16_t* pr = pos_rank + (int64_t)p * K;
-  const ArgMin ma = ranked_scan(inv, ra, pr, freq_rank, K, full, l16);
-  const ArgMin mt = ranked_scan(inv + K, rt, pr, freq_rank, K, full, l16);
-  if (l16 == 0) {
-    T0[task] = idx0[(int64_t)q * K + ma.i];
-    T1[task] = idx1[(int64_t)q * K + mt.i];
-  }
+  const int64_t task0 = (int64_t)blockIdx.x * 16;
+  const int q = (int)(task0 / K);
+  const int64_t row = (int64_t)q * K;
+  const FuseOps g{rank0 + row, rank1 + row, freq_rank, pos_rank + (task0 - row) * K, idx0 + row, idx1 + row};
+  if (staged) fuse_tasks<2>(stage_fusion<2>(inv + 2 * K, g, K), K, inv, &bad, T0 + task0, T1 + task0);
+  else fuse_tasks<2>(g, K, inv, &bad, T0 + task0, T1 + task0);
 }
 
 __global__ __launch_bounds__(256) void fuse_best_ranked_one_kernel(const int16_t* __restrict__ rank,
                                                                    const int32_t* __restrict__ idx,
                                                                    const int16_t* __restrict__ pos_rank,
                                                                    const int16_t* __restrict__ freq_rank, int Q, int K,
-                                                                   int32_t* __restrict__ T) {
+                                                                   int staged, int32_t* __restrict__ T) {
   extern __shared__ __attribute__((aligned(16))) int16_t inv[];
   __shared__ int bad;
-  const int tid = threadIdx.x, l16 = tid & 15;
-  const int64_t task = (int64_t)blockIdx.x * 16 + (tid >> 4);
-  const int q = (int)(((int64_t)blockIdx.x * 16) / K);
-  const int p = (int)(task - (int64_t)q * K);
-  const int16_t* rk = rank + (int64_t)q * K;
-  const bool full = inverse_ranks<1>(rk, nullptr, K, inv, &bad);
-  const ArgMin m = ranked_scan(inv, rk, pos_rank + (int64_t)p * K, freq_rank, K, full, l16);
-  if (l16 == 0) T[task] = idx[(int64_t)q * K + m.i];
+  const int64_t task0 = (int64_t)blockIdx.x * 16;
+  const int q = (int)(task0 / K);
+  const int64_t row = (int64_t)q * K;
+  const FuseOps g{rank + row, nullptr, freq_rank, pos_rank + (task0 - row) * K, idx + row, nullptr};
+  if (staged) fuse_tasks<1>(stage_fusion<1>(inv + K, g, K), K, inv, &bad, T + task0, nullptr);
+  else fuse_tasks<1>(g, K, inv, &bad, T + task0, nullptr);
 }
 
 struct TailArgs {
@@ -401,21 +454,39 @@
   int s_last, off_last;
 };
 
-__device__ __forceinline__ const float* cand_block(const TailArgs& A, int which, int ci, int* pay_base) {
+struct GridTabs {
+  const int32_t *cidx0, *pslot0, *cidx1, *pslot1;
+};
+__device__ __forceinline__ GridTabs grid_global(const TailArgs& A) { return GridTabs{A.cidx0, A.pslot0, A.cidx1, A.pslot1}; }
+#define QPG_GRID_LDS 256
+struct GridRegs {
+  int c0, p0, c1, p1;
+  __device__ __forceinline__ void load(const TailArgs& A, int g) {
+    c0 = p0 = c1 = p1 = 0;
+    if (g >= 0 && g < A.G0) { c0 = A.cidx0[g]; p0 = A.pslot0[g]; }
+    if (g >= 0 && g < A.G1) { c1 = A.cidx1[g]; p1 = A.pslot1[g]; }
+  }
+  __device__ __forceinline__ void store(int32_t* lds, int g) const {
+    if (g >= 0 && g < 64) { lds[g] = c0; lds[64 + g] = p0; lds[128 + g] = c1; lds[192 + g] = p1; }
+  }
+};
+__device__ __forceinline__ GridTabs grid_lds(const int32_t* lds) { return GridTabs{lds, lds + 64, lds + 128, lds + 192}; }
+
+__device__ __forceinline__ const float* cand_block(const TailArgs& A, const GridTabs& gr, int which, int ci, int* pay_base) {
   const int G = which ? A.G1 : A.G0;
   const int cc = ci < 0 ? 0 : ci;
   const int j = cc / G, g = cc - j * G;
-  const int ps = (which ? A.pslot1 : A.pslot0)[g];
-  *pay_base = j * A.code_ld + (which ? A.cidx1 : A.cidx0)[g];
+  const int ps = (which ? gr.pslot1 : gr.pslot0)[g];
+  *pay_base = j * A.code_ld + (which ? gr.cidx1 : gr.cidx0)[g];
   return A.phase + ((int64_t)j * A.Tp + ps) * 16;
 }
 
-__device__ __forceinline__ unsigned int gate_eval(const TailArgs& A, int q, int p, const float* prev, int lane) {
-  const int K = A.K;
+__device__ __forceinline__ unsigned int gate_eval(const TailArgs& A, const GridTabs& gr, const int32_t* t0q,
+                                                  const int32_t* t1q, int p, const float* prev, int lane) {
   const int k = (lane >> 2) & 1, l = lane & 3;
-  const int ck = (k ? A.T1 : A.T0)[(int64_t)q * K + p];
+  const int ck = (k ? t1q : t0q)[p];
   int pb_unused;
-  const float* head = cand_block(A, k, ck, &pb_unused);
+  const float* head = cand_block(A, gr, k, ck, &pb_unused);
   float xa[32], xb[32];
   float sa = 0.f, sb = 0.f;
 #pragma unroll
@@ -451,9 +522,10 @@
   return (unsigned int)((p << 1) | fi);
 }
 
-__device__ __forceinline__ const float* gate_prev(const TailArgs& A, const GateGeom& geo, int s, int kp, int ci, int* p) {
+__device__ __forceinline__ const float* gate_prev(const TailArgs& A, const GridTabs& gr, const GateGeom& geo, int s, int kp,
+                                                  int ci, int* p) {
   int pb;
-  const float* prev = cand_block(A, kp, ci, &pb) + 384;
+  const float* prev = cand_block(A, gr, kp, ci, &pb) + 384;
   *p = A.code[pb + (s == 0 ? geo.off_last : A.step_codes - 1)];
   return prev;
 }
@@ -470,6 +542,7 @@
   const bool first = q == chain * Qc;
   if (first && sigma != 0) return;
   const int s = q % A.steps;
+  const GridTabs gr = grid_global(A);
   int p;
   const float* prev;
   if (first) {
@@ -477,12 +550,13 @@
   } else {
     const int pp = sigma >> 1, kp = sigma & 1;
     const int ci = (kp ? A.T1 : A.T0)[(int64_t)(q - 1) * K + pp];
-    prev = gate_prev(A, geo, s, kp, ci, &p);
-  }
-  const unsigned int g = gate_eval(A, q, p, prev, lane);
+    prev = gate_prev(A, gr, geo, s, kp, ci, &p);
+  }
+  const unsigned int g = gate_eval(A, gr, A.T0 + (int64_t)q * K, A.T1 + (int64_t)q * K, p, prev, lane);
   if (live && (lane & 7) == 0) Gt[task] = (uint16_t)g;
 }
 
+#define GD_KMAX 512
 #define GD_SLOTS 2048
 #define GD_THREADS 1024
 __global__ __launch_bounds__(GD_THREADS) void gate_table_dedup_kernel(TailArgs A, GateGeom geo, uint16_t* __restrict__ Gt) {
@@ -490,6 +564,8 @@
   __shared__ unsigned short val[GD_SLOTS];
   __shared__ unsigned short ulist[GD_SLOTS];
   __shared__ int n_u;
+  __shared__ __attribute__((aligned(16))) int32_t trow[4 * GD_KMAX];
+  __shared__ int32_t s_grid[QPG_GRID_LDS];
   const int K = A.K, Qc = A.M * A.steps, tid = threadIdx.x, lane = tid & 63;
   const int q = blockIdx.x, chain = q / Qc, s = q % A.steps;
   uint16_t* out = Gt + (int64_t)q * 2 * K;
@@ -497,15 +573,24 @@
     if (tid < 8) {
       int p;
       const float* prev = chain_seed(A, chain, &p);
-      const unsigned int g = gate_eval(A, q, p, prev, lane);
+      const unsigned int g = gate_eval(A, grid_global(A), A.T0 + (int64_t)q * K, A.T1 + (int64_t)q * K, p, prev, lane);
       if (tid == 0) out[0] = (uint16_t)g;
     }
     return;
   }
+  const int half = K >> 1, tab = tid >= half;
+  int4 piece = make_int4(0, 0, 0, 0);
+  if (tid < K) piece = reinterpret_cast<const int4*>((tab ? A.T1 : A.T0) + (int64_t)(q - 1) * K)[tid - tab * half];
+  GridRegs gregs;
+  gregs.load(A, tid - (GD_THREADS - 64));
   for (int i = tid; i < GD_SLOTS; i += GD_THREADS) key[i] = 0;
   if (tid == 0) n_u = 0;
+  if (tid < K) reinterpret_cast<int4*>(trow)[tid] = piece;
+  gregs.store(s_grid, tid - (GD_THREADS - 64));
+  const GridTabs gr = grid_lds(s_grid);
+  const int32_t *t0p = trow, *t0q = trow + K, *t1p = trow + 2 * K, *t1q = trow + 3 * K;
   __syncthreads();
-  constexpr int PER = 2 * 512 / GD_THREADS;
+  constexpr int PER = 2 * GD_KMAX / GD_THREADS;
   int slot[PER];
 #pragma unroll
   for (int u = 0; u < PER; ++u) {
@@ -513,7 +598,7 @@
     slot[u] = -1;
     if (sigma < 2 * K) {
       const int pp = sigma >> 1, kp = sigma & 1;
-      const int ci = (kp ? A.T1 : A.T0)[(int64_t)(q - 1) * K + pp];
+      const int ci = (kp ? t1p : t0p)[pp];
       const int kv = (((ci < 0 ? 0 : ci) << 1) | kp) + 1;
       unsigned int h = ((unsigned int)kv * 2654435761u) >> 21;
       for (;;) {
@@ -533,8 +618,8 @@
   for (int u = tid >> 3; u < nu; u += GD_THREADS >> 3) {
     const int h = ulist[u], kv = key[h] - 1;
     int p;
-    const float* prev = gate_prev(A, geo, s, kv & 1, kv >> 1, &p);
-    const unsigned int g = gate_eval(A, q, p, prev, lane);
+    const float* prev = gate_prev(A, gr, geo, s, kv & 1, kv >> 1, &p);
+    const unsigned int g = gate_eval(A, gr, t0q, t1q, p, prev, lane);
     if ((lane & 7) == 0) val[h] = (unsigned short)g;
   }
   __syncthreads();
@@ -545,31 +630,47 @@
 
 #define QPG_CHASE_QMAX 2048
 
-template <class Chase>
-__device__ __forceinline__ void chase_windows(uint16_t* gl, const uint16_t* __restrict__ Gt, int M, int per_w, Chase chase) {
-  const int tid = threadIdx.x, nt = blockDim.x;
-  auto stage = [&](int w, int first, int step) {
-    const int4* src = reinterpret_cast<const int4*>(Gt + (int64_t)w * per_w);
-    int4* dst = reinterpret_cast<int4*>(gl + (size_t)(w & 1) * per_w);
-    for (int v = first; v < per_w / 8; v += step) dst[v] = src[v];
-  };
-  stage(0, tid, nt);
+__device__ __forceinline__ void copy16(i32x4* dst, const i32x4* __restrict__ src, int n, int first, int step) {
+  for (int b = first; b < n; b += 8 * step) {
+    i32x4 r[8];
+#pragma unroll
+    for (int u = 0; u < 8; ++u) r[u] = src[b + u * step < n ? b + u * step : b];
+#pragma unroll
+    for (int u = 0; u < 8; ++u)
+      if (b + u * step < n) dst[b + u * step] = r[u];
+  }
+}
+
+template <class Under, class Chase>
+__device__ __forceinline__ void chase_windows(uint16_t* gl, const uint16_t* __restrict__ Gt, int M, int per_w, int W,
+                                              Under under, Chase chase) {
+  const int tid = threadIdx.x, nt = blockDim.x, n_w = per_w / 8;
+  const i32x4* src = reinterpret_cast<const i32x4*>(Gt);
+  i32x4* ring = reinterpret_cast<i32x4*>(gl);
+  const bool whole = M <= W;
+  copy16(ring, src, (whole ? M : W - 1) * n_w, tid, nt);
+  under();
   __syncthreads();
+  int slot = 0, ahead = W - 1;
   for (int w = 0; w < M; ++w) {
-    if (tid >= 64 && w + 1 < M) stage(w + 1, tid - 64, nt - 64);
-    chase(w, gl + (size_t)(w & 1) * per_w);
-    __syncthreads();
-  }
-}
-
-__device__ __forceinline__ void walk_epilogue(const TailArgs& A, const uint16_t* sig, int* bad, int Q, int K) {
+    if (!whole && tid >= 64 && w + W - 1 < M)
+      copy16(ring + (size_t)ahead * n_w, src + (size_t)(w + W - 1) * n_w, n_w, tid - 64, nt - 64);
+    chase(w, gl + (size_t)slot * per_w);
+    if (!whole && w + 1 < M) __syncthreads();
+    slot = slot + 1 == W ? 0 : slot + 1;
+    ahead = ahead + 1 == W ? 0 : ahead + 1;
+  }
+}
+
+__device__ __forceinline__ void walk_epilogue(const TailArgs& A, const GridTabs& gr, const uint16_t* sig, int* bad, int Q,
+                                              int K) {
   const int tid = threadIdx.x, nt = blockDim.x;
   for (int i = tid; i < Q * 32; i += nt) {
     const int q = i >> 5, v = i & 31;
     const int sg = sig[q], p = sg >> 1, fi = sg & 1;
     const int ci = (fi ? A.T1 : A.T0)[(int64_t)q * K + p];
     int pb;
-    const float* blk = cand_block(A, fi, ci, &pb) + 384;
+    const float* blk = cand_block(A, gr, fi, ci, &pb) + 384;
     reinterpret_cast<f32x4*>(A.out_phase + (int64_t)q * 128)[v] = reinterpret_cast<const f32x4*>(blk)[v];
     if (v == 0) {
       A.out_vote[q] = fi;
@@ -582,15 +683,16 @@
     const int sg = sig[q], p = sg >> 1, fi = sg & 1;
     const int ci = (fi ? A.T1 : A.T0)[(int64_t)q * K + p];
     int pb;
-    cand_block(A, fi, ci, &pb);
+    cand_block(A, gr, fi, ci, &pb);
     A.out_codes[i] = A.code[pb + c % A.step_codes];
   }
   write_status_pair(A, *bad);
 }
 
-__global__ __launch_bounds__(1024) void gate_chase_kernel(TailArgs A, const uint16_t* __restrict__ Gt) {
+__global__ __launch_bounds__(1024) void gate_chase_kernel(TailArgs A, int ring, const uint16_t* __restrict__ Gt) {
   extern __shared__ __attribute__((aligned(16))) uint16_t gl[];
   __shared__ uint16_t sig[QPG_CHASE_QMAX];
+  __shared__ int32_t s_grid[QPG_GRID_LDS];
   __shared__ int bad_s;
   const int K = A.K, Q = A.M * A.steps, tid = threadIdx.x;
   const int per_w = A.steps * 2 * K;
@@ -604,8 +706,10 @@
   A.out_codes += (int64_t)chain * A.M * A.codes_per_window;
   A.out_status += (int64_t)chain * A.status_stride;
   if (tid == 0) bad_s = 0;
+  const int gt = tid - ((int)blockDim.x - 64);
+  GridRegs gregs;
   int sigma = 0;
-  chase_windows(gl, Gt, A.M, per_w, [&](int w, const uint16_t* g) {
+  chase_windows(gl, Gt, A.M, per_w, ring, [&]() { gregs.load(A, gt); }, [&](int w, const uint16_t* g) {
     if (tid == 0) {
       for (int s = 0; s < A.steps; ++s) {
         sigma = (w == 0 && s == 0) ? g[0] : g[s * 2 * K + sigma];
@@ -613,7 +717,9 @@
       }
     }
   });
-  walk_epilogue(A, sig, &bad_s, Q, K);
+  gregs.store(s_grid, gt);
+  __syncthreads();
+  walk_epilogue(A, grid_lds(s_grid), sig, &bad_s, Q, K);
 }
 
 #define QPG_TAKES_PER_BLOCK 64
@@ -627,11 +733,11 @@
   int p;
   const float* prev = chain_seed(A, take, &p);
   p = p < 0 ? 0 : (p >= A.K ? A.K - 1 : p);
-  const unsigned int g = gate_eval(A, 0, p, prev, lane);
+  const unsigned int g = gate_eval(A, grid_global(A), A.T0, A.T1, p, prev, lane);
   if (live && (lane & 7) == 0) step0[take] = (uint16_t)g;
 }
 
-__global__ __launch_bounds__(1024) void gate_chase_takes_kernel(int M, int steps, int K, int n_takes,
+__global__ __launch_bounds__(1024) void gate_chase_takes_kernel(int M, int steps, int K, int n_takes, int ring,
                                                                 const uint16_t* __restrict__ Gt,
                                                                 const uint16_t* __restrict__ step0,
                                                                 uint16_t* __restrict__ trail) {
@@ -641,7 +747,7 @@
   const int take = blockIdx.x * QPG_TAKES_PER_BLOCK + tid;
   const bool chaser = tid < QPG_TAKES_PER_BLOCK && take < n_takes;
   int sigma = chaser ? step0[take] : 0;
-  chase_windows(gl, Gt, M, per_w, [&](int w, const uint16_t* g) {
+  chase_windows(gl, Gt, M, per_w, ring, []() {}, [&](int w, const uint16_t* g) {
     if (chaser) {
       for (int s = 0; s < steps; ++s) {
         if (w | s) sigma = g[s * 2 * K + sigma];
@@ -653,22 +759,32 @@
 
 __global__ __launch_bounds__(256) void takes_epilogue_kernel(TailArgs A, int n_takes, const uint16_t* __restrict__ trail) {
   __shared__ uint16_t sig[QPG_CHASE_QMAX];
+  __shared__ int32_t s_grid[QPG_GRID_LDS];
   __shared__ int bad_s;
   const int K = A.K, Q = A.M * A.steps, tid = threadIdx.x, nt = blockDim.x;
   const int take = blockIdx.x;
+  GridRegs gregs;
+  gregs.load(A, tid);
   A.out_phase += (int64_t)take * Q * 128;
   A.out_vote += (int64_t)take * Q;
   A.out_codes += (int64_t)take * A.M * A.codes_per_window;
   A.out_status += (int64_t)take * A.status_stride;
   if (tid == 0) bad_s = 0;
   for (int q = tid; q < Q; q += nt) sig[q] = trail[(int64_t)q * n_takes + take];
+  gregs.store(s_grid, tid);
   __syncthreads();
-  walk_epilogue(A, sig, &bad_s, Q, K);
+  walk_epilogue(A, grid_lds(s_grid), sig, &bad_s, Q, K);
 }
 
 __global__ void status_only_kernel(int32_t* out_status, const int32_t* guard_flags) {
   out_status[0] = 0;
   out_status[1] = guard_flags ? guard_flags[0] : 0;
+}
+
+static int fuse_staged(int K, const void* a, const void* b, const void* c, const void* d, const void* e = nullptr,
+                       const void* f = nullptr) {
+  const uintptr_t bits = (uintptr_t)a | (uintptr_t)b | (uintptr_t)c | (uintptr_t)d | (uintptr_t)e | (uintptr_t)f;
+  return K <= QPG_FUSE_STAGED_KMAX && (bits & 15) == 0;
 }
 
 extern "C" int qpg_fuse_best_ranked(qpg_ctx* ctx, void* stream, const int16_t* rank, const int32_t* idx,
@@ -676,8 +792,9 @@
   QPG_REQUIRE(ctx && rank && idx && pos_rank && freq_rank && T, "qpg_fuse_best_ranked: null pointer");
   QPG_REQUIRE(Q > 0 && K > 0 && (K % 16) == 0 && K <= 4096 && ((int64_t)Q * K) / 16 < 0x7fffffffll,
               "qpg_fuse_best_ranked: K %% 16 == 0, K <= 4096");
-  hipLaunchKernelGGL(fuse_best_ranked_one_kernel, dim3((unsigned)(((int64_t)Q * K) / 16)), dim3(256), 2 * (size_t)K,
-                     qpg_stream(stream), rank, idx, pos_rank, freq_rank, Q, K, T);
+  const int staged = fuse_staged(K, rank, idx, pos_rank, freq_rank);
+  hipLaunchKernelGGL(fuse_best_ranked_one_kernel, dim3((unsigned)(((int64_t)Q * K) / 16)), dim3(256),
+                     (size_t)(staged ? 42 : 2) * K, qpg_stream(stream), rank, idx, pos_rank, freq_rank, Q, K, staged, T);
   QPG_LAUNCH_CHECK("fuse_best_ranked_one_kernel");
   return QPG_OK;
 }
@@ -686,6 +803,8 @@
   int codes_per_window;
   GateGeom gate;
   size_t lds_cand;
+  size_t lds_window;
+  int ring;
   size_t lds_chase;
   bool tabulated;
 };
@@ -696,25 +815,71 @@
   const int last_idx = g.codes_per_window - 1;
   g.gate = GateGeom{last_idx / 4, last_idx % 4};
   g.lds_cand = (size_t)2 * steps * K * sizeof(int32_t);
-  g.lds_chase = (size_t)2 * steps * 2 * K * sizeof(uint16_t);
+  g.lds_window = (size_t)steps * 2 * K * sizeof(uint16_t);
+  g.ring = 2;
+  g.lds_chase = 2 * g.lds_window;
   g.tabulated = !serial_walk && g.gate.s_last == steps - 1 && 2 * K <= 65536 && Qc <= QPG_CHASE_QMAX &&
-                g.lds_chase <= 64 * 1024 && ((steps * 2 * K) % 8) == 0;
+                2 * g.lds_window <= 64 * 1024 && ((steps * 2 * K) % 8) == 0;
   return g;
 }
 
-static int walk_lds_ok(const char* name, const void* kernel, size_t dyn) {
-  if (dyn <= 56 * 1024) return QPG_OK;
-  hipFuncAttributes fa;
-  if (hipFuncGetAttributes(&fa, kernel) != hipSuccess) {
-    qpg_set_error("%s: cannot read the kernel's attributes", name);
+enum { WALK_LDS_SERIAL = 0, WALK_LDS_CHASE = 1, WALK_LDS_TAKES = 2 };
+struct WalkKernel {
+  int slot;
+  const char* name;
+  const void* fn;
+};
+static WalkKernel walk_kernel(int slot) {
+  if (slot == WALK_LDS_SERIAL) return {slot, "match_walk_kernel", reinterpret_cast<const void*>(match_walk_kernel)};
+  if (slot == WALK_LDS_CHASE) return {slot, "gate_chase_kernel", reinterpret_cast<const void*>(gate_chase_kernel)};
+  return {slot, "gate_chase_takes_kernel", reinterpret_cast<const void*>(gate_chase_takes_kernel)};
+}
+
+static int walk_static_lds(qpg_ctx* ctx, const WalkKernel& k, int* bytes) {
+  auto& rec = ctx->walk_lds[k.slot];
+  if (rec.static_bytes < 0) {
+    hipFuncAttributes fa;
+    if (hipFuncGetAttributes(&fa, k.fn) != hipSuccess) {
+      qpg_set_error("%s: cannot read the kernel's attributes", k.name);
+      return QPG_EHIP;
+    }
+    rec.static_bytes = (int)fa.sharedSizeBytes;
+  }
+  *bytes = rec.static_bytes;
+  return QPG_OK;
+}
+
+static int walk_lds_ok(qpg_ctx* ctx, const WalkKernel& k, size_t dyn) {
+  auto& rec = ctx->walk_lds[k.slot];
+  if (dyn <= rec.granted) return QPG_OK;
+  int st = 0;
+  const int rc = walk_static_lds(ctx, k, &st);
+  if (rc != QPG_OK) return rc;
+  if ((size_t)st + dyn > 64 * 1024 &&
+      hipFuncSetAttribute(k.fn, hipFuncAttributeMaxDynamicSharedMemorySize, (int)dyn) != hipSuccess) {
+    (void)hipGetLastError();
+    qpg_set_error("%s: cannot raise the dynamic LDS limit to %zu bytes", k.name, dyn);
     return QPG_EHIP;
   }
-  if (fa.sharedSizeBytes + dyn > 64 * 1024 &&
-      hipFuncSetAttribute(kernel, hipFuncAttributeMaxDynamicSharedMemorySize, (int)dyn) != hipSuccess) {
-    qpg_set_error("%s: cannot raise the dynamic LDS limit to %zu bytes", name, dyn);
-    return QPG_EHIP;
-  }
+  rec.granted = dyn;
   return QPG_OK;
+}
+
+static int chase_ring(qpg_ctx* ctx, bool takes, int M, WalkGeom* g) {
+  const WalkKernel k = walk_kernel(takes ? WALK_LDS_TAKES : WALK_LDS_CHASE);
+  int st = 0;
+  int rc = walk_static_lds(ctx, k, &st);
+  if (rc != QPG_OK) return rc;
+  const int cap = ctx->opt[QPG_OPT_CHASE_RING_WINDOWS];
+  const size_t room = ctx->lds_per_block > st ? (size_t)(ctx->lds_per_block - st) : 0;
+  int64_t W = (int64_t)(room / g->lds_window);
+  if (W > M) W = M;
+  if (cap >= 2 && W > cap) W = cap;
+  if (W < 2) W = 2;
+  if (W > 2 && walk_lds_ok(ctx, k, (size_t)W * g->lds_window) != QPG_OK) W = 2;
+  g->ring = (int)W;
+  g->lds_chase = (size_t)W * g->lds_window;
+  return walk_lds_ok(ctx, k, g->lds_chase);
 }
 
 struct WalkArgs {
@@ -755,7 +920,7 @@
               "qpg_match_steps: bad size");
   const int Qc = M * steps;
   const int Q = Qc * n_chains;
-  const WalkGeom geo = walk_geom(serial_walk, steps, K, Qc);
+  WalkGeom geo = walk_geom(serial_walk, steps, K, Qc);
   QPG_REQUIRE(geo.lds_cand <= 96 * 1024, "qpg_match_steps: steps*K too large for the LDS gate tables");
   if (M == 0) {
     hipLaunchKernelGGL(status_only_kernel, dim3(1), dim3(1), 0, qpg_stream(stream), a.out_status, a.guard_flags);
@@ -770,20 +935,18 @@
   QPG_REQUIRE(n_takes <= 0 || (a.takes_ws && a.takes_ws_bytes >= qpg_match_steps_takes_ws_bytes(n_takes, M, steps)),
               "qpg_match_steps_takes: workspace too small (qpg_match_steps_takes_ws_bytes)");
   {
-    int rc = QPG_OK;
-    if (!geo.tabulated) rc = walk_lds_ok("match_walk_kernel", reinterpret_cast<const void*>(match_walk_kernel), geo.lds_cand);
-    else if (n_takes > 0)
-      rc = walk_lds_ok("gate_chase_takes_kernel", reinterpret_cast<const void*>(gate_chase_takes_kernel), geo.lds_chase);
-    else rc = walk_lds_ok("gate_chase_kernel", reinterpret_cast<const void*>(gate_chase_kernel), geo.lds_chase);
+    const int rc = geo.tabulated ? chase_ring(ctx, n_takes > 0, M, &geo)
+                                 : walk_lds_ok(ctx, walk_kernel(WALK_LDS_SERIAL), geo.lds_cand);
     if (rc != QPG_OK) return rc;
   }
   int32_t* T0 = a.gate_tables;
   int32_t* T1 = a.gate_tables + (int64_t)Q * K;
   if (prefused) {
   } else if (mode == 0 && (K % 16) == 0 && K <= 4096) {
-    hipLaunchKernelGGL(fuse_best_ranked_kernel, dim3((unsigned)(((int64_t)Q * K) / 16)), dim3(256), 4 * (size_t)K,
-                       qpg_stream(stream), a.aud_rank, a.aud_idx, a.txt_rank, a.txt_idx, a.pos_rank, a.freq_rank, Q, K, T0,
-                       T1);
+    const int staged = fuse_staged(K, a.aud_rank, a.aud_idx, a.txt_rank, a.txt_idx, a.pos_rank, a.freq_rank);
+    hipLaunchKernelGGL(fuse_best_ranked_kernel, dim3((unsigned)(((int64_t)Q * K) / 16)), dim3(256),
+                       (size_t)(staged ? 50 : 4) * K, qpg_stream(stream), a.aud_rank, a.aud_idx, a.txt_rank, a.txt_idx,
+                       a.pos_rank, a.freq_rank, Q, K, staged, T0, T1);
     QPG_LAUNCH_CHECK("fuse_best_ranked_kernel");
   } else {
     dim3 grid((unsigned)(((int64_t)Q * K + 3) / 4), 1);
@@ -811,7 +974,7 @@
   uint16_t* gtab = reinterpret_cast<uint16_t*>(a.gate_tables + (int64_t)2 * Q * K);
   const int64_t lanes = (int64_t)Q * 2 * K * 8;
   const int dedup_from = ctx->opt[QPG_OPT_GATE_DEDUP_FROM_CHAINS];
-  if (dedup_from > 0 && n_chains >= dedup_from && K <= 512) {
+  if (dedup_from > 0 && n_chains >= dedup_from && K <= GD_KMAX) {
     hipLaunchKernelGGL(gate_table_dedup_kernel, dim3((unsigned)Q), dim3(GD_THREADS), 0, qpg_stream(stream), A, geo.gate,
                        gtab);
     QPG_LAUNCH_CHECK("gate_table_dedup_kernel");
@@ -832,7 +995,7 @@
     if (stages & 2) {
       hipLaunchKernelGGL(gate_chase_takes_kernel,
                          dim3((unsigned)((n_takes + QPG_TAKES_PER_BLOCK - 1) / QPG_TAKES_PER_BLOCK)), dim3(1024),
-                         geo.lds_chase, qpg_stream(stream), M, steps, K, n_takes, (const uint16_t*)gtab,
+                         geo.lds_chase, qpg_stream(stream), M, steps, K, n_takes, geo.ring, (const uint16_t*)gtab,
                          (const uint16_t*)step0, trail);
       QPG_LAUNCH_CHECK("gate_chase_takes_kernel");
     }
@@ -843,10 +1006,17 @@
     }
     return QPG_OK;
   }
-  hipLaunchKernelGGL(gate_chase_kernel, dim3(n_chains), dim3(1024), geo.lds_chase, qpg_stream(stream), A,
+  hipLaunchKernelGGL(gate_chase_kernel, dim3(n_chains), dim3(1024), geo.lds_chase, qpg_stream(stream), A, geo.ring,
                      (const uint16_t*)gtab);
   QPG_LAUNCH_CHECK("gate_chase_kernel");
   return QPG_OK;
+}
+
+extern "C" int qpg_match_steps_ring_windows(qpg_ctx* ctx, int M, int steps, int K, int takes) {
+  if (!ctx || M < 1 || steps < 1 || steps * 4 > 64 || K < 1 || K > 64 * QPG_KMAX_PER_LANE || (K % 4) != 0) return 0;
+  WalkGeom geo = walk_geom(false, steps, K, M * steps);
+  if (!geo.tabulated || chase_ring(ctx, takes != 0, M, &geo) != QPG_OK) return 0;
+  return geo.ring;
 }
 
 extern "C" int qpg_match_steps(qpg_ctx* ctx, void* stream, const int16_t* aud_rank, const int32_t* aud_idx,
```

After: 5.352 million frames/s. -2.1%, worse.
